# Beryl2000/SE-UNet-AirSeg

Hardware: AMD Instinct MI355X
Metric: voxels/sec SE-UNet fwd+bwd, 128^3 patch (higher is better)
Workload: dtype bf16

## Files before the change

include/seunet_hip.h:

```cpp
#ifndef SEUNET_HIP_H
#define SEUNET_HIP_H
#include <stddef.h>

#ifdef __cplusplus
extern "C" {
#endif

#ifndef SEUNET_F32
#define SEUNET_F32 0
#define SEUNET_BF16 1
#define SEUNET_F16 2
#endif
#define SEUNET_CONV_MFMA 0
#define SEUNET_CONV_NAIVE 1
#define SEUNET_CONV_MARCH 2
#define SEUNET_CONV_TILED 3

typedef void* seunet_stream_t;
typedef struct seunet_dims { int n, d, h, w; } seunet_dims;

int seunet_version(void);
const char* seunet_last_error(void);
int seunet_init(int device);

int seunet_pack_cl(int dtype, const float* in_ncdhw, int c, void* out_cl, int c_pad, seunet_dims dims, seunet_stream_t s);
int seunet_unpack_cl(int dtype, const void* in_cl, int c, float* out_ncdhw, seunet_dims dims, seunet_stream_t s);

size_t seunet_conv_wpack_bytes(int dtype, int taps, int cin, int cout);
int seunet_conv_pack_weights(int dtype, const float* w, int taps, int cin, int cout, int transpose_flip, void* wpack, seunet_stream_t s);
int seunet_conv_stats_slots(int impl, int taps, int dilation, seunet_dims dims);
int seunet_conv3d_fwd(int dtype, int impl, int taps, int dilation, int nsrc, const void* const* src, const int* src_c,
                      int cin, const void* weights, int transpose_flip, const float* bias, int ndst, void* const* dst,
                      const int* dst_c, const int* dst_accumulate, double* stats_partial, seunet_dims dims, seunet_stream_t s);
int seunet_conv3d_stream_supported(int dtype, int dilation, int src_c, int dst_c);
size_t seunet_conv3d_stream_wpack_bytes(int src_c);
int seunet_conv3d_stream_slots(int dilation, seunet_dims dims);
int seunet_conv3d_stream_pack(int dtype, const float* w, int cin_w, int cout_w, int transpose_flip, int src_c, int dst_c, void* wpack,
                              seunet_stream_t s);
int seunet_conv3d_stream(int dtype, int dilation, const void* src, int src_c, const void* wpack, const float* bias, void* dst, int dst_c,
                         int dst_accumulate, double* stats_partial, seunet_dims dims, seunet_stream_t s);
int seunet_conv3d_march_supported(int dtype, int dilation, int nsrc, const int* src_c, int ndst, const int* dst_c);
size_t seunet_conv3d_march_wpack_bytes(int cin, int cout);
int seunet_conv3d_march_slots(int dilation, int cin, int cout, seunet_dims dims);
int seunet_conv3d_march_pack(int dtype, const float* w, int cin_w, int cout_w, int transpose_flip, int cin, int cout, void* wpack,
                             seunet_stream_t s);
int seunet_conv3d_march(int dtype, int dilation, int nsrc, const void* const* src, const int* src_c, const void* wpack, const float* bias,
                        int ndst, void* const* dst, const int* dst_c, const int* dst_accumulate, double* stats_partial, seunet_dims dims,
                        seunet_stream_t s);
int seunet_conv3d_wgrad_stream_supported(int dtype, int dilation, int x_c, int dy_c);
size_t seunet_conv3d_wgrad_stream_workspace_bytes(int x_c, int dy_c, int dilation, seunet_dims dims);
int seunet_conv3d_wgrad_stream(int dtype, int dilation, const void* x, int x_c, int cin, const void* dy, int dy_c, int cout, float* dw,
                               void* workspace, size_t workspace_bytes, seunet_dims dims, seunet_stream_t s);
size_t seunet_conv3d_wgrad_workspace_bytes(int taps, int cin, int cout);
int seunet_conv3d_wgrad(int dtype, int impl, int taps, int dilation, int nsrc, const void* const* src, const int* src_c,
                        int cin, const void* dy, int cout, float* dw, void* workspace, size_t workspace_bytes,
                        seunet_dims dims, seunet_stream_t s);

int seunet_epilogue_slots(seunet_dims dims);
int seunet_channel_stats(int dtype, const void* t, int c, double* partial, seunet_dims dims, seunet_stream_t s);
int seunet_stats_finalize(const double* partial, int slots, int c, int n, long long count, float eps, int mode,
                          float* out_a, float* out_b, seunet_stream_t s);

int seunet_gate_epilogue_fwd(int dtype, const void* raw, const float* mean, const float* rstd, int c, const float* w_se,
                             const float* w_se2, const float* w_side, const float* b_side, float slope, void* e_out,
                             float* side_out, float* level_map, int level_accumulate, const float* head_w,
                             const float* drop, int drop_stride, seunet_dims dims, seunet_stream_t s);
int seunet_gate_epilogue_bwd(int dtype, const void* raw, const float* mean, const float* rstd, int c, const float* w_se,
                             const float* w_se2, const float* w_side, const float* b_side, float slope, const void* g_e,
                             const float* g_side, const float* g_level, const float* head_w, const float* drop,
                             int drop_stride, const float* m1, const float* m2, void* draw_out, double* stat_partial,
                             float* pgrad_partial, seunet_dims dims, seunet_stream_t s);
int seunet_pgrad_reduce(const float* pgrad_partial, int records, int c, float* dw_se, float* dw_se2, float* dw_side,
                        float* db_side, float* dhead_w, seunet_stream_t s);
int seunet_gate_bwd_finalize(const double* stat_partial, int slots, int c, int n, long long count, float* m1, float* m2,
                             const float* pgrad_partial, int records, float* dw_se, float* dw_se2, float* dw_side,
                             float* db_side, float* dhead_w, seunet_stream_t s);

int seunet_cat_epilogue_fwd(int dtype, const void* raw, const float* mean, const float* rstd, const void* raw2,
                            const float* mean2, const float* rstd2, int c, float slope, void* out, seunet_dims dims,
                            seunet_stream_t s);
int seunet_cat_epilogue_bwd(int dtype, const void* g_out, const void* raw, const float* mean, const float* rstd,
                            const void* raw2, const float* mean2, const float* rstd2, int c, float slope,
                            const float* m1, const float* m2, const float* m1b, const float* m2b, void* dx, void* dx2,
                            double* stat_partial, double* stat_partial2, seunet_dims dims, seunet_stream_t s);

int seunet_xbranch_moment_slots(seunet_dims dims);
int seunet_xbranch_moments(int dtype, const void* x_in, double* partial , seunet_dims dims, seunet_stream_t s);
int seunet_xbranch_stats(const double* partial, int slots, const float* w2, int c, int in_channel, int n, long long count,
                         float eps, float* mean2, float* rstd2, double* moments_out , seunet_stream_t s);
int seunet_cat_epilogue_fwd_x(int dtype, const void* raw, const float* mean, const float* rstd, const void* x_in,
                              const float* w2, int in_channel, const float* mean2, const float* rstd2, int c, float slope,
                              void* out, seunet_dims dims, seunet_stream_t s);
int seunet_cat_epilogue_bwd_x(int dtype, const void* g_out, const void* raw, const float* mean, const float* rstd,
                              const void* x_in, const float* w2, int in_channel, const float* mean2, const float* rstd2,
                              int c, float slope, const float* m1, const float* m2, const float* m1b, const float* m2b,
                              void* dx, double* stat_partial, double* stat_partial2, double* xw_partial, seunet_dims dims,
                              seunet_stream_t s);
int seunet_cat_epilogue_fwd_x_pool(int dtype, const void* raw, const float* mean, const float* rstd, const void* x_in,
                                   const float* w2, int in_channel, const float* mean2, const float* rstd2, int c, float slope,
                                   void* out, void* pooled, unsigned int* argmax, seunet_dims dims, seunet_stream_t s);
int seunet_cat_epilogue_bwd_x_pool(int dtype, const void* g_out, const void* raw, const float* mean, const float* rstd,
                                   const void* x_in, const float* w2, int in_channel, const float* mean2, const float* rstd2,
                                   int c, float slope, const float* m1, const float* m2, const float* m1b, const float* m2b,
                                   void* dx, double* stat_partial, double* stat_partial2, double* xw_partial,
                                   const unsigned int* pool_argmax, const void* pool_g, seunet_dims dims, seunet_stream_t s);
int seunet_cat_xgrad_finalize(const double* xw_partial, const double* stat_partial2, int slots, const double* moments,
                              const float* w2, int c, int in_channel, int n, float eps, float* dw, seunet_stream_t s);

int seunet_maxpool_fwd(int dtype, const void* in, int c, void* out, seunet_dims in_dims, seunet_stream_t s);
int seunet_maxpool_bwd(int dtype, const void* in, const void* g_out, int c, void* g_in, int accumulate,
                       seunet_dims in_dims, seunet_stream_t s);
int seunet_upsample2_fwd(int dtype, const void* in, int c, void* out, seunet_dims in_dims, seunet_stream_t s);
int seunet_upsample2_bwd(int dtype, const void* g_out, int c, void* g_in, int accumulate, seunet_dims in_dims,
                         seunet_stream_t s);
int seunet_side_upsample(const float* side, int c, int scale, float* out_ncdhw, int c_total, int c_off,
                         seunet_dims low_dims, seunet_stream_t s);

int seunet_head_fwd(const float* const* level_maps, int nlevels, const float* bias, float* pred, seunet_dims dims,
                    seunet_stream_t s);
size_t seunet_head_bwd_tmp_floats(seunet_dims dims);
int seunet_head_bwd(const float* g_pred, float* const* g_levels, int nlevels, float* tmp, float* g_bias,
                    seunet_dims dims, seunet_stream_t s);

#define SEUNET_LOSS_DICE 1
#define SEUNET_LOSS_GUL 2
#define SEUNET_LOSS_ATR 4
int seunet_loss_partial_floats(void);
int seunet_loss_sums(const float* pred, int apply_sigmoid, const float* target, const float* weight, const float* skel,
                     long long n, float* partial, double* sums, int terms, seunet_stream_t s);
int seunet_loss_value(const double* sums0, double c_dice0, double c_gul0, double c_atr0, const double* sums1, double c_dice1,
                      double c_gul1, double c_atr1, float* value, seunet_stream_t s);
int seunet_loss_grad(const float* pred, int apply_sigmoid, const float* target, const float* weight, const float* skel,
                     long long n, const double* sums, float c_dice, float c_gul, float c_atr, float g_scale,
                     const float* g_scale_dev, float* g_pred, seunet_stream_t s);

int seunet_loss_sample_partial_floats(int batch);
int seunet_loss_sums_per_sample(const float* pred, int apply_sigmoid, const float* target, const float* weight, const float* skel,
                                int batch, long long n_per_sample, float* partial, double* sums, int terms, seunet_stream_t s);
int seunet_loss_sample_values(const double* sums, int batch, double c_dice, double c_gul, double c_atr, float* values,
                              seunet_stream_t s);

size_t seunet_cldice_workspace_bytes(long long volumes, int n0, int n1, int n2, int iters, int save);
int seunet_cldice_partial_doubles(void);
int seunet_soft_skeleton(const float* x, long long volumes, int n0, int n1, int n2, int iters, float* out, int save, void* workspace,
                         size_t workspace_bytes, seunet_stream_t s);
int seunet_cldice_sums(const float* skel_pred, const float* target, const float* skel_target, const float* pred, long long n,
                       double* partial, double* sums, seunet_stream_t s);
int seunet_cldice_value(const double* sums, double smooth, float* value, double* scalars, seunet_stream_t s);
int seunet_cldice_backward(const float* target, const float* skel_target, const double* sums, double smooth, const float* g_dev,
                           long long volumes, int n0, int n1, int n2, int iters, float* grad, void* workspace, size_t workspace_bytes,
                           seunet_stream_t s);
int seunet_cldice_counts(const unsigned char* skel_pred, const unsigned char* label, const unsigned char* skel_label,
                         const unsigned char* pred, long long n, unsigned long long* counts, seunet_stream_t s);

int seunet_pool_select(const float* new_keys, int batch, float* keys, long long* seq, long long* state, int capacity, int* slots_out,
                       seunet_stream_t s);
int seunet_pool_scatter(const int* slots_dev, int batch, int capacity, long long voxels, const float* data, const float* label,
                        const float* weight, const float* skel, float* pool_data, unsigned char* pool_label, float* pool_weight,
                        unsigned char* pool_skel, seunet_stream_t s);
int seunet_pool_gather(const int* slots_host, int n, int capacity, long long voxels, const float* pool_data,
                       const unsigned char* pool_label, const float* pool_weight, const unsigned char* pool_skel, float* data_out,
                       float* label_out, float* weight_out, float* skel_out, seunet_stream_t s);

int seunet_adamw_step(float* const* params, const float* const* grads, float* const* exp_avg, float* const* exp_avg_sq,
                      const long long* counts, int n_tensors, double lr, double beta1, double beta2, double eps,
                      double weight_decay, int step, int maximize, seunet_stream_t s);
int seunet_adamw_step_gated(float* const* params, const float* const* grads, float* const* exp_avg, float* const* exp_avg_sq,
                            const long long* counts, const int* steps, float* const* skipped, int n_tensors, double lr,
                            double beta1, double beta2, double eps, double weight_decay, int maximize, const int* skip_flag,
                            float* table, seunet_stream_t s);

#define SEUNET_IMG_I16 0
#define SEUNET_IMG_F32 1
#define SEUNET_W_F16 0
#define SEUNET_W_F32 1
#define SEUNET_W_F64 2
int seunet_crop_batch(const void* img, int img_dtype, const unsigned char* label, const void* weight, int weight_dtype,
                      const unsigned char* skeleton, int d, int h, int w, int cube, int ncrop, const int* starts, const int* aug,
                      double weight_exponent, int f64_math, float* data_out, float* label_out, float* weight_out, float* skel_out,
                      seunet_stream_t s);
int seunet_hu_two_channel(const void* img, int img_dtype, long long nvox, int f64_math, float* out, seunet_stream_t s);

int seunet_window_gather(const float* volume, int c, int x, int y, int z, int cube, int nwin, const int* starts, float* out,
                         seunet_stream_t s);
int seunet_window_accumulate(const float* logits, int apply_sigmoid, int nwin, const int* starts, int cube, double* acc, int x, int y,
                             int z, seunet_stream_t s);
int seunet_window_finalize(const double* acc, int x, int y, int z, int cube, int nx, const int* xs, int ny, const int* ys, int nz,
                           const int* zs, int dup0, double* out, seunet_stream_t s);

#define SEUNET_DTI_F64 0
// ... 176 lines not shown
```

se-unet-airseg_amd/_lib.py:

```python
from __future__ import annotations

import ctypes as C
import os
from typing import Optional, Sequence

_HERE = os.path.dirname(os.path.abspath(__file__))
LIB_PATH = os.environ.get("SEUNET_LIB") or os.path.join(_HERE, "libseunet_hip.so")

F32, BF16, F16 = 0, 1, 2
CONV_MFMA, CONV_NAIVE, CONV_MARCH, CONV_TILED = 0, 1, 2, 3
LOSS_NSUMS = 7
DTI_F64, DTI_F32 = 0, 1
CC_EVALUATION, CC_MAXIMUM_3D, CC_LARGEST_FILLED = 0, 1, 2
MORPH_DILATE, MORPH_ERODE_BORDER0, MORPH_ERODE_BORDER1, MORPH_CLOSE = 0, 1, 2, 3


class Dims(C.Structure):
    _fields_ = [("n", C.c_int), ("d", C.c_int), ("h", C.c_int), ("w", C.c_int)]


class NetDesc(C.Structure):
    _fields_ = [("batch", C.c_int), ("in_channel", C.c_int), ("n_classes", C.c_int),
                ("d", C.c_int), ("h", C.c_int), ("w", C.c_int), ("width_mult", C.c_int),
                ("dtype", C.c_int), ("conv_impl", C.c_int),
# ... 1 lines not shown


KERNEL_NAIVE, KERNEL_TILED, KERNEL_STREAM, KERNEL_MARCH, KERNEL_WGRAD1X1 = range(5)
KERNEL_NAMES = ("Naive", "Tiled", "Stream", "March", "Wgrad1x1")


class ConvInfo(C.Structure):
    _fields_ = [("name", C.c_char * 16), ("taps", C.c_int), ("dilation", C.c_int), ("level", C.c_int), ("dims", Dims),
                ("nsrc", C.c_int), ("src_c", C.c_int * 3), ("src_is_input", C.c_int * 3), ("cin", C.c_int), ("cout", C.c_int),
                ("need_dgrad", C.c_int), ("fwd", C.c_int), ("dgrad", C.c_int), ("wgrad", C.c_int),
                ("x_name", C.c_char * 16), ("x_materialised", C.c_int), ("x_fwd", C.c_int), ("x_wgrad", C.c_int),
                ("src_dist", C.c_longlong)]


_vp, _i, _f, _ll, _sz, _d =C.c_void_p, C.c_int, C.c_float, C.c_longlong, C.c_size_t, C.c_double
_pp = C.POINTER(C.c_void_p)
_ip = C.POINTER(C.c_int)

PROTOTYPES = {
    "seunet_version": (_i, []),
    "seunet_last_error": (C.c_char_p, []),
    "seunet_pack_cl": (_i, [_i, _vp, _i, _vp, _i, Dims, _vp]),
    "seunet_unpack_cl": (_i, [_i, _vp, _i, _vp, Dims, _vp]),
    "seunet_conv_wpack_bytes": (_sz, [_i, _i, _i, _i]),
    "seunet_conv_pack_weights": (_i, [_i, _vp, _i, _i, _i, _i, _vp, _vp]),
    "seunet_conv_stats_slots": (_i, [_i, _i, _i, Dims]),
    "seunet_conv3d_fwd": (_i, [_i, _i, _i, _i, _i, _pp, _ip, _i, _vp, _i, _vp, _i, _pp, _ip, _ip, _vp, Dims, _vp]),
    "seunet_conv3d_stream_supported": (_i, [_i, _i, _i, _i]),
    "seunet_conv3d_stream_wpack_bytes": (_sz, [_i]),
    "seunet_conv3d_stream_slots": (_i, [_i, Dims]),
    "seunet_conv3d_stream_pack": (_i, [_i, _vp, _i, _i, _i, _i, _i, _vp, _vp]),
    "seunet_conv3d_stream": (_i, [_i, _i, _vp, _i, _vp, _vp, _vp, _i, _i, _vp, Dims, _vp]),
    "seunet_conv3d_march_supported": (_i, [_i, _i, _i, _ip, _i, _ip]),
    "seunet_conv3d_march_wpack_bytes": (_sz, [_i, _i]),
    "seunet_conv3d_march_slots": (_i, [_i, _i, _i, Dims]),
    "seunet_conv3d_march_pack": (_i, [_i, _vp, _i, _i, _i, _i, _i, _vp, _vp]),
    "seunet_conv3d_march": (_i, [_i, _i, _i, _pp, _ip, _vp, _vp, _i, _pp, _ip, _ip, _vp, Dims, _vp]),
    "seunet_conv3d_wgrad_stream_supported": (_i, [_i, _i, _i, _i]),
    "seunet_conv3d_wgrad_stream_workspace_bytes": (_sz, [_i, _i, _i, Dims]),
    "seunet_conv3d_wgrad_stream": (_i, [_i, _i, _vp, _i, _i, _vp, _i, _i, _vp, _vp, _sz, Dims, _vp]),
    "seunet_conv3d_wgrad_workspace_bytes": (_sz, [_i, _i, _i]),
    "seunet_conv3d_wgrad": (_i, [_i, _i, _i, _i, _i, _pp, _ip, _i, _vp, _i, _vp, _vp, _sz, Dims, _vp]),
    "seunet_epilogue_slots": (_i, [Dims]),
    "seunet_channel_stats": (_i, [_i, _vp, _i, _vp, Dims, _vp]),
    "seunet_stats_finalize": (_i, [_vp, _i, _i, _i, _ll, _f, _i, _vp, _vp, _vp]),
    "seunet_gate_epilogue_fwd": (_i, [_i, _vp, _vp, _vp, _i, _vp, _vp, _vp, _vp, _f, _vp, _vp, _vp, _i, _vp, _vp, _i, Dims, _vp]),
    "seunet_gate_epilogue_bwd": (_i, [_i, _vp, _vp, _vp, _i, _vp, _vp, _vp, _vp, _f, _vp, _vp, _vp, _vp, _vp, _i, _vp, _vp, _vp, _vp, _vp, Dims, _vp]),
    "seunet_pgrad_reduce": (_i, [_vp, _i, _i, _vp, _vp, _vp, _vp, _vp, _vp]),
    "seunet_gate_bwd_finalize": (_i, [_vp, _i, _i, _i, _ll, _vp, _vp, _vp, _i, _vp, _vp, _vp, _vp, _vp, _vp]),
    "seunet_cat_epilogue_fwd": (_i, [_i, _vp, _vp, _vp, _vp, _vp, _vp, _i, _f, _vp, Dims, _vp]),
    "seunet_cat_epilogue_bwd": (_i, [_i, _vp, _vp, _vp, _vp, _vp, _vp, _vp, _i, _f, _vp, _vp, _vp, _vp, _vp, _vp, _vp, _vp, Dims, _vp]),
    "seunet_maxpool_fwd": (_i, [_i, _vp, _i, _vp, Dims, _vp]),
    "seunet_maxpool_bwd": (_i, [_i, _vp, _vp, _i, _vp, _i, Dims, _vp]),
    "seunet_upsample2_fwd": (_i, [_i, _vp, _i, _vp, Dims, _vp]),
    "seunet_upsample2_bwd": (_i, [_i, _vp, _i, _vp, _i, Dims, _vp]),
    "seunet_side_upsample": (_i, [_vp, _i, _i, _vp, _i, _i, Dims, _vp]),
    "seunet_head_fwd": (_i, [_pp, _i, _vp, _vp, Dims, _vp]),
    "seunet_head_bwd_tmp_floats": (_sz, [Dims]),
    "seunet_head_bwd": (_i, [_vp, _pp, _i, _vp, _vp, Dims, _vp]),
    "seunet_loss_partial_floats": (_i, []),
    "seunet_loss_sums": (_i, [_vp, _i, _vp, _vp, _vp, _ll, _vp, _vp, _i, _vp]),
    "seunet_loss_value": (_i, [_vp, _d, _d, _d, _vp, _d, _d, _d, _vp, _vp]),
    "seunet_loss_grad": (_i, [_vp, _i, _vp, _vp, _vp, _ll, _vp, _f, _f, _f, _f, _vp, _vp, _vp]),
    "seunet_loss_sample_partial_floats": (_i, [_i]),
    "seunet_loss_sums_per_sample": (_i, [_vp, _i, _vp, _vp, _vp, _i, _ll, _vp, _vp, _i, _vp]),
    "seunet_loss_sample_values": (_i, [_vp, _i, _d, _d, _d, _vp, _vp]),
    "seunet_cldice_workspace_bytes": (_sz, [_ll, _i, _i, _i, _i, _i]),
    "seunet_cldice_partial_doubles": (_i, []),
    "seunet_soft_skeleton": (_i, [_vp, _ll, _i, _i, _i, _i, _vp, _i, _vp, _sz, _vp]),
    "seunet_cldice_sums": (_i, [_vp, _vp, _vp, _vp, _ll, _vp, _vp, _vp]),
    "seunet_cldice_value": (_i, [_vp, _d, _vp, _vp, _vp]),
    "seunet_cldice_backward": (_i, [_vp, _vp, _vp, _d, _vp, _ll, _i, _i, _i, _i, _vp, _vp, _sz, _vp]),
    "seunet_cldice_counts": (_i, [_vp, _vp, _vp, _vp, _ll, _vp, _vp]),
    "seunet_pool_select":(_i, [_vp, _i, _vp, _vp, _vp, _i, _vp, _vp]),
    "seunet_pool_scatter": (_i, [_vp, _i, _i, _ll, _vp, _vp, _vp, _vp, _vp, _vp, _vp, _vp, _vp]),
    "seunet_pool_gather": (_i, [_ip, _i, _i, _ll, _vp, _vp, _vp, _vp, _vp, _vp, _vp, _vp, _vp]),
    "seunet_xbranch_moment_slots": (_i, [Dims]),
    "seunet_xbranch_moments": (_i, [_i, _vp, _vp, Dims, _vp]),
    "seunet_xbranch_stats": (_i, [_vp, _i, _vp, _i, _i, _i, _ll, _f, _vp, _vp, _vp, _vp]),
    "seunet_cat_epilogue_fwd_x": (_i, [_i, _vp, _vp, _vp, _vp, _vp, _i, _vp, _vp, _i, _f, _vp, Dims, _vp]),
    "seunet_cat_epilogue_bwd_x": (_i, [_i, _vp, _vp, _vp, _vp, _vp, _vp, _i, _vp, _vp, _i, _f, _vp, _vp, _vp, _vp, _vp, _vp, _vp, _vp, Dims, _vp]),
    "seunet_cat_epilogue_fwd_x_pool": (_i, [_i, _vp, _vp, _vp, _vp, _vp, _i, _vp, _vp, _i, _f, _vp, _vp, _vp, Dims, _vp]),
    "seunet_cat_epilogue_bwd_x_pool": (_i, [_i, _vp, _vp, _vp, _vp, _vp, _vp, _i, _vp, _vp, _i, _f, _vp, _vp, _vp, _vp, _vp, _vp, _vp, _vp, _vp, _vp, Dims, _vp]),
    "seunet_cat_xgrad_finalize": (_i, [_vp, _vp, _i, _vp, _vp, _i, _i, _i, _f, _vp, _vp]),
    "seunet_cc_workspace_bytes": (_sz, [_i, _i, _i]),
    "seunet_largest_component": (_i, [_vp, _i, _i, _i, _i, _vp, _vp, _vp, _sz, _vp]),
    "seunet_metric_out_bytes": (_sz, [_i]),
    "seunet_metric_sums": (_i, [_vp, _vp, _vp, _vp, _ll, _i, _vp, _sz, _vp]),
    "seunet_value_counts": (_i, [_vp, _ll, _i, _vp, _vp]),
    "seunet_shift_clamp": (_i, [_vp, _ll, _i, _i, _i, _i, _vp, _vp]),
    "seunet_get_l_workspace_bytes": (_sz, [_i, _i, _i]),
    "seunet_get_l": (_i, [_vp, _i, _i, _i, _d, _i, _vp, _vp, _sz, _vp]),
    "seunet_mask_combine": (_i, [_vp, _vp, _ll, _i, _vp, _vp]),
    "seunet_mask_box": (_i, [_vp, _i, _i, _i, _vp, _vp]),
    "seunet_crop3d": (_i, [_vp, _i, _i, _i, _i, _ip, _vp, _vp]),
    "seunet_crop_batch": (_i, [_vp, _i, _vp, _vp, _i, _vp, _i, _i, _i, _i, _i, _ip, _ip, C.c_double, _i, _vp, _vp, _vp, _vp, _vp]),
    "seunet_hu_two_channel": (_i, [_vp, _i, _ll, _i, _vp, _vp]),
    "seunet_window_gather": (_i, [_vp, _i, _i, _i, _i, _i, _i, _ip, _vp, _vp]),
    "seunet_window_accumulate": (_i, [_vp, _i, _i, _ip, _i, _vp, _i, _i, _i, _vp]),
    "seunet_window_finalize": (_i, [_vp, _i, _i, _i, _i, _i, _ip, _i, _ip, _i, _ip, _i, _vp, _vp]),
    "seunet_dti_workspace_bytes": (_sz, [_i, _i, _i]),
    "seunet_dti": (_i, [_vp, _i, _i, _i, C.c_double, C.c_double, _i, _vp, _vp, _sz, _vp]),
    "seunet_edt_workspace_bytes": (_sz, [_i, _i, _i]),
    "seunet_edt": (_i, [_vp, _i, _i, _i, _vp, _vp, _vp, _vp, _vp, _sz, _vp]),
    "seunet_edt_sampling_workspace_bytes": (_sz, [_i, _i, _i]),
    "seunet_edt_sampling": (_i, [_vp, _i, _i, _i, _d, _d, _d, _vp, _vp, _vp, _vp, _vp, _sz, _vp]),
    "seunet_mask_bits": (_i, [_vp, _ll, _vp, _vp]),
    "seunet_hard_mining_masks": (_i, [_vp, _vp, _vp, _i, _i, _i, _vp, _vp, _vp]),
    "seunet_lib_weight_workspace_bytes": (_sz, [_i, _i, _i]),
    "seunet_lib_weight": (_i, [_vp, _i, _i, _i, _vp, _vp, _vp, _sz, _vp]),
    "seunet_break_weight_workspace_bytes": (_sz, [_i, _i, _i]),
    "seunet_break_weight": (_i, [_vp, _vp, _vp, _i, _i, _i, _vp, _vp, _vp, _vp, _sz, _vp]),
    "seunet_skeleton_workspace_bytes": (_sz, [_i, _i, _i]),
    "seunet_skeletonize": (_i, [_vp, _i, _i, _i, _vp, _vp, _vp, _sz, _vp]),
    "seunet_skeleton_branches_workspace_bytes": (_sz, [_i, _i, _i]),
    "seunet_skeleton_branches": (_i, [_vp, _i, _i, _i, _i, _vp, _vp, _vp, _vp, _sz, _vp]),
    "seunet_parse_assign_workspace_bytes": (_sz, [_i, _i, _i]),
    "seunet_parse_assign": (_i, [_vp, _vp, _vp, _i, _i, _i, _vp, _vp, _vp, _sz, _vp]),
    "seunet_label_stats_max_num": (_i, []),
    "seunet_label_stats": (_i, [_vp, _i, _i, _i, _i, _vp, _vp, _vp, _vp]),
    "seunet_relabel": (_i, [_vp, _ll, _vp, _i, _vp, _vp]),
    "seunet_binary_morph_workspace_bytes": (_sz, [_i, _i, _i]),
    "seunet_binary_morph": (_i, [_vp, _i, _i, _i, _i, _vp, _vp, _sz, _vp]),
    "seunet_fill_holes": (_i, [_vp, _i, _i, _i, _vp, _vp, _sz, _vp]),
    "seunet_slice_moments": (_i, [_vp, _i, _i, _i, _i, _vp, _vp]),
    "seunet_scatter_labels": (_i, [_vp, _vp, _ll, _ll, _vp, _vp, _vp, _vp]),
    "seunet_mesh_workspace_bytes": (_sz, [_i, _i, _i]),
    "seunet_mesh_count": (_i, [_vp, _i, _i, _i, C.POINTER(_ll), C.POINTER(_ll), _vp, _sz, _vp]),
    "seunet_mesh_emit": (_i, [_i, _i, _i, _d, _ll, _ll, _vp, _vp, _vp, _sz, _vp]),
    "seunet_mesh_label_workspace_bytes": (_sz, [_i, _i, _i]),
    "seunet_mesh_label_sort_bytes": (_sz, [_ll, _ll]),
    "seunet_mesh_label_count": (_i, [_vp, _i, _i, _i, _i, C.POINTER(_ll), C.POINTER(_ll), _ip, _ip, _vp, _vp, _i, _vp, _sz, _vp]),
    "seunet_mesh_label_emit": (_i, [_vp, _i, _i, _i, _i, _d, _ll, _ll, _vp, _vp, _vp, _sz, _vp, _sz, _vp]),
    "seunet_branch_stats": (_i, [_vp, _vp, _vp, _i, _i, _i, _i] + [_vp] * 11 + [_vp]),
    "seunet_branch_wall_stats": (_i, [_vp, _vp, _vp, _i, _i, _i, _i, _d, _d, _d, _vp, _vp, _vp, _vp, _vp, _vp]),
    "seunet_surface_workspace_bytes": (_sz, [_i, _i, _i]),
    "seunet_surface_count": (_i, [_vp, _vp, _i, _i, _i, C.POINTER(_ll), C.POINTER(_ll), _ip, _vp, _sz, _vp]),
    "seunet_surface_emit_workspace_bytes": (_sz, [_i, _i, _i]),
    "seunet_surface_emit": (_i, [_i, _i, _i, _ip, _d, _d, _d, _ll, _ll, _vp, _vp, _vp, _sz, _vp, _sz, _vp]),
    "seunet_surface_summary_bytes": (_sz, [_i]),
    "seunet_surface_summary": (_i, [_vp, _ll, _ll, C.POINTER(_d), _i, _vp, _vp]),
    "seunet_select_ranks_workspace_bytes": (_sz, [_i]),
    "seunet_select_ranks": (_i, [_vp, _ll, C.POINTER(_ll), C.POINTER(_ll), C.POINTER(_ll), _i, _vp, _vp, _sz, _vp]),
    "seunet_mesh_coord_sums": (_i, [_vp, _i, _i, _i, _vp, _vp]),
    "seunet_mesh_adjacency_workspace_bytes": (_sz, [_ll, _ll]),
    "seunet_mesh_adjacency": (_i, [_vp, _ll, _ll, _vp, _vp, _ll, _vp, _vp, _vp, _sz, _vp]),
    "seunet_mesh_smooth": (_i, [_vp, _ll, _vp, _vp, _vp, _i, _f, _vp, _vp, _vp]),
    "seunet_mesh_affine": (_i, [_vp, _ll, C.POINTER(_f), C.POINTER(_f), _vp, _vp]),
    "seunet_mesh_stl_records": (_i, [_vp, _ll, _vp, _ll, C.POINTER(_f), C.POINTER(_f), _vp, _vp, _vp]),
    "seunet_adamw_step": (_i, [_vp, _vp, _vp, _vp, _vp, _i, C.c_double, C.c_double, C.c_double, C.c_double, C.c_double, _i, _i, _vp]),
    "seunet_adamw_step_gated": (_i, [_vp, _vp, _vp, _vp, _vp, _vp, _vp, _i, C.c_double, C.c_double, C.c_double, C.c_double, C.c_double,
                                     _i, _vp, _vp, _vp]),
    "seunet_net_param_count": (_i, [C.POINTER(NetDesc)]),
    "seunet_net_param_info": (_i, [C.POINTER(NetDesc), _i, C.c_char_p, _i, _ip, _ip]),
    "seunet_net_workspace_bytes": (_sz, [C.POINTER(NetDesc)]),
    "seunet_net_forward": (_i, [C.POINTER(NetDesc), _pp, _vp, _vp, _vp, _vp, _vp, _vp, _sz, _vp]),
    "seunet_prof_enable": (_i, [_i]),
    "seunet_prof_enable_filtered": (_i, [C.c_char_p]),
    "seunet_prof_report": (_i, [C.c_char_p, _sz]),
    "seunet_init": (_i, [_i]),
    "seunet_net_forward_capture": (_i, [C.POINTER(NetDesc), _pp, _vp, _vp, _vp, _vp, _vp, _vp, _sz, _vp, C.POINTER(C.c_void_p)]),
    "seunet_graph_launch": (_i, [_vp, _vp]),
    "seunet_graph_destroy": (_i, [_vp]),
    "seunet_net_read_tensor": (_i, [C.POINTER(NetDesc), _pp, _vp, _sz, C.c_char_p, _i, _vp, _ip, _vp]),
    "seunet_net_conv_info": (_i, [C.POINTER(NetDesc), _i, C.POINTER(ConvInfo)]),
    "seunet_net_backward": (_i, [C.POINTER(NetDesc), _pp, _vp, _vp, _vp, _vp, _pp, _vp, _sz, _vp]),
# ... 63 lines not shown
```

se-unet-airseg_amd/csrc/abi.cpp:

```cpp
#include "seunet_common.h"
#include "epilogue.h"
#include "volume.h"
#include "wgrad.h"
#include "../../include/seunet_hip.h"

using namespace seunet;

static inline Dims D(seunet_dims d) { return Dims{d.n, d.d, d.h, d.w}; }
static inline hipStream_t S(seunet_stream_t s) { return reinterpret_cast<hipStream_t>(s); }

static int make_src(int nsrc, const void* const* src, const int* src_c, SrcList& l) {
  SEUNET_CHECK(nsrc >= 1 && nsrc <= 3 && src && src_c, "bad source list");
  l = SrcList{};
  l.n = nsrc;
  for (int i = 0; i < nsrc; ++i) { l.ptr[i] = src[i]; l.C[i] = src_c[i]; }
  return 0;
}

namespace seunet { extern unsigned long long* g_conv_debug; }

extern "C" {

int seunet_debug_set_buffer(void* p) { seunet::g_conv_debug = reinterpret_cast<unsigned long long*>(p); return 0; }
int seunet_debug_upsample2_form(int dtype, int c, seunet_dims dims, int backward) { return upsample2_form(dtype, c, D(dims), backward != 0); }
// ... 135 lines not shown
                        seunet_stream_t s) {
  SrcList sl;
  if (int e = make_src(nsrc, src, src_c, sl)) return e;
  SEUNET_CHECK(dy && dw, "conv3d_wgrad: null tensor");
  if (impl == SEUNET_CONV_NAIVE) return launch_wgrad_naive(dtype, taps, dilation, sl, cin, dy, cout, dw, D(dims), S(s));
  SEUNET_CHECK(workspace, "conv3d_wgrad: null workspace");
  const ConvKernel k = impl == SEUNET_CONV_MARCH ? (taps == 1 ? ConvKernel::Wgrad1x1 : ConvKernel::March)
                       : impl == SEUNET_CONV_TILED ? ConvKernel::Tiled
                                                   : wgrad_kernel(dtype, taps, dilation, sl, cin, cout, D(dims), sl.gap());
  return run_wgrad(k, dtype, taps, dilation, sl, cin, dy, cout, dw, workspace, workspace_bytes, D(dims), S(s));
}

int seunet_epilogue_slots(seunet_dims dims) { return epi_partials(D(dims)); }
int seunet_channel_stats(int dtype, const void* t, int c, double* partial, seunet_dims dims, seunet_stream_t s) {
  SEUNET_CHECK(t && partial, "channel_stats: null tensor");
  return launch_channel_stats(dtype, t, c, partial, D(dims), S(s));
}
int seunet_stats_finalize(const double* partial, int slots, int c, int n, long long count, float eps, int mode, float* out_a,
                          float* out_b, seunet_stream_t s) {
  SEUNET_CHECK(partial && out_a && out_b && slots >= 1 && count >= 1, "stats_finalize: bad argument");
  return launch_stats_finalize(partial, slots, c, n, count, eps, mode, out_a, out_b, S(s));
}

int seunet_gate_epilogue_fwd(int dtype, const void* raw, const float* mean, const float* rstd, int c, const float* w_se,
                             const float* w_se2, const float* w_side, const float* b_side, float slope, void* e_out,
                             float* side_out, float* level_map, int level_accumulate, const float* head_w, const float* drop,
                             int drop_stride, seunet_dims dims, seunet_stream_t s) {
  SEUNET_CHECK(raw && mean && rstd && w_se && w_side && b_side && e_out, "gate_epilogue_fwd: null tensor");
  SEUNET_CHECK(!level_map || head_w, "gate_epilogue_fwd: level_map needs head_w");
  const GateBlock b{{raw, mean, rstd}, c, {w_se, w_se2, w_side, b_side, slope}};
  SseHead h{side_out, level_map, level_accumulate, head_w, drop, drop_stride};
  return launch_sse_fwd(dtype, b, e_out, h, D(dims), S(s));
}
int seunet_gate_epilogue_bwd(int dtype, const void* raw, const float* mean, const float* rstd, int c, const float* w_se,
                             const float* w_se2, const float* w_side, const float* b_side, float slope, const void* g_e,
                             const float* g_side, const float* g_level, const float* head_w, const float* drop, int drop_stride,
                             const float* m1, const float* m2, void* draw_out, double* stat_partial, float* pgrad_partial,
                             seunet_dims dims, seunet_stream_t s) {
  SEUNET_CHECK(raw && mean && rstd && w_se && w_side && b_side, "gate_epilogue_bwd: null tensor");
  SEUNET_CHECK(!g_level || head_w, "gate_epilogue_bwd: g_level needs head_w");
  const GateBlock b{{raw, mean, rstd}, c, {w_se, w_se2, w_side, b_side, slope}};
  SseBwdIn g{g_e, g_side, g_level};
  SseHead h{nullptr, nullptr, 0, head_w, drop, drop_stride};
  if (m1 == nullptr) return launch_sse_bwd_sums(dtype, b, g, h, {stat_partial, pgrad_partial}, D(dims), S(s));
  return launch_sse_bwd_apply(dtype, b, g, h, {m1, m2, draw_out}, D(dims), S(s));
}
int seunet_pgrad_reduce(const float* pgrad_partial, int records, int c, float* dw_se, float* dw_se2, float* dw_side,
                        float* db_side, float* dhead_w, seunet_stream_t s) {
  SEUNET_CHECK(pgrad_partial && records >= 1, "pgrad_reduce: bad argument");
  return launch_pgrad_reduce(pgrad_partial, records, c, dw_se, dw_se2, dw_side, db_side, dhead_w, S(s));
}
int seunet_gate_bwd_finalize(const double* stat_partial, int slots, int c, int n, long long count, float* m1, float* m2,
                             const float* pgrad_partial, int records, float* dw_se, float* dw_se2, float* dw_side,
                             float* db_side, float* dhead_w, seunet_stream_t s) {
  SEUNET_CHECK(stat_partial && m1 && m2 && pgrad_partial && slots >= 1 && n >= 1 && count >= 1, "gate_bwd_finalize: bad argument");
  SEUNET_CHECK(c % 8 == 0 && c >= 8 && c <= 128 && (c & (c - 1)) == 0, "channel count %d must be a power of two in [8,128]", c);
  SEUNET_CHECK(records == n * slots, "gate_bwd_finalize: records=%d, pass A wrote n * slots = %d", records, n * slots);
  return launch_gate_bwd_finalize(stat_partial, slots, c, n, count, m1, m2, pgrad_partial, records, dw_se, dw_se2, dw_side,
                                  db_side, dhead_w, S(s));
}
static int cat_epilogue_bwd(int dtype, const CatBlock& b, const void* g_out, const PoolGrad& pool, const float* m1, const float* m2,
                            const float* m1b, const float* m2b, void* dx, void* dx2, double* stat_partial, double* stat_partial2,
                            double* xw_partial, seunet_dims dims, seunet_stream_t s) {
  if (m1 == nullptr) return launch_cat_bwd_sums(dtype, b, g_out, pool, {stat_partial, stat_partial2, xw_partial}, D(dims), S(s));
  return launch_cat_bwd_apply(dtype, b, g_out, pool, {m1, m2, m1b, m2b, dx, dx2, nullptr, 0}, D(dims), S(s));
}
int seunet_cat_epilogue_fwd(int dtype, const void* raw, const float* mean, const float* rstd, const void* raw2,
                            const float* mean2, const float* rstd2, int c, float slope, void* out, seunet_dims dims,
                            seunet_stream_t s) {
  SEUNET_CHECK(raw && mean && rstd && out && (!raw2 || (mean2 && rstd2)), "cat_epilogue_fwd: null tensor");
  const CatBlock b{{raw, mean, rstd}, {raw2 ? Branch2::Stored : Branch2::None, raw2, mean2, rstd2, nullptr, 0}, c, slope};
  return launch_cat_fwd(dtype, b, out, PoolOut{}, D(dims), S(s));
}
int seunet_cat_epilogue_bwd(int dtype, const void* g_out, const void* raw, const float* mean, const float* rstd,
                            const void* raw2, const float* mean2, const float* rstd2, int c, float slope, const float* m1,
                            const float* m2, const float* m1b, const float* m2b, void* dx, void* dx2, double* stat_partial,
                            double* stat_partial2, seunet_dims dims, seunet_stream_t s) {
  SEUNET_CHECK(g_out && raw && mean && rstd, "cat_epilogue_bwd: null tensor");
  SEUNET_CHECK(!raw2 || (mean2 && rstd2), "cat_epilogue_bwd: second branch incomplete");
  const CatBlock b{{raw, mean, rstd}, {raw2 ? Branch2::Stored : Branch2::None, raw2, mean2, rstd2, nullptr, 0}, c, slope};
  return cat_epilogue_bwd(dtype, b, g_out, PoolGrad{}, m1, m2, m1b, m2b, dx, dx2, stat_partial, stat_partial2, nullptr, dims, s);
}

int seunet_maxpool_fwd(int dtype, const void* in, int c, void* out, seunet_dims d, seunet_stream_t s) {
  SEUNET_CHECK(in && out, "maxpool_fwd: null tensor");
  return launch_maxpool_fwd(dtype, in, c, out, D(d), S(s));
}
int seunet_maxpool_bwd(int dtype, const void* in, const void* g_out, int c, void* g_in, int accumulate, seunet_dims d,
                       seunet_stream_t s) {
  SEUNET_CHECK(in && g_out && g_in, "maxpool_bwd: null tensor");
  return launch_maxpool_bwd(dtype, in, g_out, c, g_in, accumulate, D(d), S(s));
}
int seunet_upsample2_fwd(int dtype, const void* in, int c, void* out, seunet_dims d, seunet_stream_t s) {
  SEUNET_CHECK(in && out, "upsample2_fwd: null tensor");
  return launch_upsample2_fwd(dtype, in, c, out, D(d), S(s));
}
int seunet_upsample2_bwd(int dtype, const void* g_out, int c, void* g_in, int accumulate, seunet_dims d, seunet_stream_t s) {
  SEUNET_CHECK(g_out && g_in, "upsample2_bwd: null tensor");
  return launch_upsample2_bwd(dtype, g_out, c, g_in, accumulate, D(d), S(s));
}
int seunet_side_upsample(const float* side, int c, int scale, float* out, int c_total, int c_off, seunet_dims low,
                         seunet_stream_t s) {
  SEUNET_CHECK(side && out && scale >= 1, "side_upsample: bad argument");
  return launch_side_upsample(side, c, scale, out, c_total, c_off, D(low), S(s));
}

int seunet_head_fwd(const float* const* level_maps, int nlevels, const float* bias, float* pred, seunet_dims d, seunet_stream_t s) {
  SEUNET_CHECK(level_maps && bias && pred, "head_fwd: null tensor");
  return launch_head_fwd(level_maps, nlevels, bias, pred, D(d), S(s));
}
size_t seunet_head_bwd_tmp_floats(seunet_dims d) { return head_bwd_tmp_floats(D(d)); }
int seunet_head_bwd(const float* g_pred, float* const* g_levels, int nlevels, float* tmp, float* g_bias, seunet_dims d,
                    seunet_stream_t s) {
  SEUNET_CHECK(g_pred && g_levels && tmp, "head_bwd: null tensor");
  return launch_head_bwd(g_pred, g_levels, nlevels, tmp, g_bias, D(d), S(s));
}

int seunet_loss_partial_floats(void) { return loss_partials() * SEUNET_LOSS_NSUMS; }
int seunet_loss_sums(const float* pred, int apply_sigmoid, const float* target, const float* weight, const float* skel,
                     long long n, float* partial, double* sums, int terms, seunet_stream_t s) {
  SEUNET_CHECK(pred && target && partial && sums && n >= 1, "loss_sums: bad argument");
  SEUNET_CHECK(terms >= 0 && terms <= 7, "loss_sums: terms=%d is not a mask of SEUNET_LOSS_DICE | _GUL | _ATR", terms);
  return launch_loss_sums(pred, apply_sigmoid, target, weight, skel, n, partial, sums, S(s), terms);
}
int seunet_loss_value(const double* sums0, double c_dice0, double c_gul0, double c_atr0, const double* sums1, double c_dice1,
                      double c_gul1, double c_atr1, float* value, seunet_stream_t s) {
  SEUNET_CHECK(sums0 && value, "loss_value: null argument");
  return launch_loss_value(sums0, c_dice0, c_gul0, c_atr0, sums1, c_dice1, c_gul1, c_atr1, value, S(s));
}
int seunet_loss_grad(const float* pred, int apply_sigmoid, const float* target, const float* weight, const float* skel,
                     long long n, const double* sums, float c_dice, float c_gul, float c_atr, float g_scale,
                     const float* g_scale_dev, float* g_pred, seunet_stream_t s) {
  SEUNET_CHECK(pred && target && sums && g_pred && n >= 1, "loss_grad: bad argument");
  return launch_loss_grad(pred, apply_sigmoid, target, weight, skel, n, sums, c_dice, c_gul, c_atr, g_scale, g_scale_dev, g_pred, S(s));
}

int seunet_loss_sample_partial_floats(int batch) {
  if (batch < 1 || batch > 65535) { fail("loss_sample_partial_floats: batch %d (1..65535)", batch); return 0; }
  return loss_sample_partials(batch) * SEUNET_LOSS_NSUMS;
}
int seunet_loss_sums_per_sample(const float* pred, int apply_sigmoid, const float* target, const float* weight, const float* skel,
                                int batch, long long n_per_sample, float* partial, double* sums, int terms, seunet_stream_t s) {
  SEUNET_CHECK(pred && target && partial && sums && n_per_sample >= 1, "loss_sums_per_sample: bad argument");
  SEUNET_CHECK(batch >= 1 && batch <= 65535, "loss_sums_per_sample: batch %d (1..65535)", batch);
  SEUNET_CHECK(terms >= 0 && terms <= 7, "loss_sums_per_sample: terms=%d is not a mask of SEUNET_LOSS_DICE | _GUL | _ATR", terms);
  return launch_loss_sums_per_sample(pred, apply_sigmoid, target, weight, skel, batch, n_per_sample, partial, sums, terms, S(s));
}
int seunet_loss_sample_values(const double* sums, int batch, double c_dice, double c_gul, double c_atr, float* values, seunet_stream_t s) {
  SEUNET_CHECK(sums && values && batch >= 1, "loss_sample_values: bad argument");
  return launch_loss_sample_values(sums, batch, c_dice, c_gul, c_atr, values, S(s));
}

size_t seunet_cldice_workspace_bytes(long long volumes, int n0, int n1, int n2, int iters, int save) {
  if (volumes < 1 || n0 < 1 || n1 < 1 || n2 < 1) { fail("cldice_workspace_bytes: empty shape (%lld volumes of (%d, %d, %d))", volumes, n0, n1, n2); return 0; }
  if (iters < 0 || iters > kCldiceMaxIters) { fail("cldice_workspace_bytes: iters=%d (0..%d)", iters, kCldiceMaxIters); return 0; }
  if ((long long)n0 * n1 * n2 >= (1ll << 31) / volumes) { fail("cldice_workspace_bytes: fewer than 2^31 voxels in all supported"); return 0; }
  return cldice_workspace_bytes(volumes, n0, n1, n2, iters, save != 0);
}
int seunet_cldice_partial_doubles(void) { return cldice_partial_doubles(); }
int seunet_soft_skeleton(const float* x, long long volumes, int n0, int n1, int n2, int iters, float* out, int save, void* workspace,
                         size_t workspace_bytes, seunet_stream_t s) {
  return launch_soft_skeleton(x, volumes, n0, n1, n2, iters, out, save != 0, workspace, workspace_bytes, S(s));
}
int seunet_cldice_sums(const float* skel_pred, const float* target, const float* skel_target, const float* pred, long long n,
                       double* partial, double* sums, seunet_stream_t s) {
  return launch_cldice_sums(skel_pred, target, skel_target, pred, n, partial, sums, S(s));
// ... 378 lines not shown
```

se-unet-airseg_amd/csrc/cat.hip:

```cpp
#include "epilogue.h"
#include "wgrad.h"
#include <type_traits>

namespace seunet {

template <bool XR>
__device__ __forceinline__ void second_branch(const float (&in8)[8], const float (&wa)[8], const float (&wb)[8], float (&x2)[8]) {
#pragma unroll
  for (int j = 0; j < 8; ++j) x2[j] = XR ? wa[j] * in8[0] + wb[j] * in8[1] : in8[j];
}

template <typename T, int LPV, bool TWO, bool XR>
__global__ void __launch_bounds__(EPI_THREADS)
cat_fwd_kernel(const T* __restrict__ raw, const float* __restrict__ mean, const float* __restrict__ rstd,
               const T* __restrict__ raw2, const float* __restrict__ mean2, const float* __restrict__ rstd2, int C, float slope,
               T* __restrict__ out, long long V, const float* __restrict__ w2x, int xic) {
  SEUNET_EPI_THREAD(LPV);
  float mu[8], rs[8], mu2[8], rs2[8], wa[8], wb[8];
#pragma unroll
  for (int j = 0; j < 8; ++j) {
    mu[j] = mean[n * C + c0 + j]; rs[j] = rstd[n * C + c0 + j];
    mu2[j] = TWO ? mean2[n * C + c0 + j] : 0.f;
    rs2[j] = TWO ? rstd2[n * C + c0 + j] : 0.f;
    wa[j] = XR ? w2x[(c0 + j) * xic] : 0.f;
// ... 4 lines not shown
  Pack8<T> nx, nx2;
  zero8p(nx); zero8p(nx2);
  if (v < V) {
    const long long o = ((long long)n * V + v) * C + c0;
    load8p(raw + o, nx);
    if (TWO) load8p(XR ? raw2 + ((long long)n * V + v) * 8 : raw2 + o, nx2);
  }
  for (; v < V; v += stride) {
    const long long o = ((long long)n * V + v) * C + c0;
    float x[8], in2[8], x2[8], y[8];
    unpack8(nx, x);
    if (TWO) { unpack8(nx2, in2); second_branch<XR>(in2, wa, wb, x2); }
    if (v + stride < V) {
      load8p(raw + o + stride * C, nx);
      if (TWO) load8p(XR ? raw2 + ((long long)n * V + v + stride) * 8 : raw2 + o + stride * C, nx2);
    }
#pragma unroll
    for (int j = 0; j < 8; ++j) y[j] = norm_lrelu(x[j], mu[j], rs[j], slope);
    if (TWO) {
#pragma unroll
      for (int j = 0; j < 8; ++j) y[j] += norm_lrelu(x2[j], mu2[j], rs2[j], slope);
    }
    store8(out + o, y);
  }
}

template <typename T, int LPV>
__global__ void __launch_bounds__(EPI_THREADS)
cat_fwd_pool_kernel(const T* __restrict__ raw, const float* __restrict__ mean, const float* __restrict__ rstd,
                    const T* __restrict__ xin, const float* __restrict__ mean2, const float* __restrict__ rstd2, int C, float slope,
                    T* __restrict__ out, T* __restrict__ pooled, int D, int H, int W, const float* __restrict__ w2x, int xic,
                    unsigned* __restrict__ argmax) {
  SEUNET_EPI_THREAD(LPV);
  float mu[8], rs[8], mu2[8], rs2[8], wa[8], wb[8];
#pragma unroll
  for (int j = 0; j < 8; ++j) {
    mu[j] = mean[n * C + c0 + j]; rs[j] = rstd[n * C + c0 + j];
    mu2[j] = mean2[n * C + c0 + j]; rs2[j] = rstd2[n * C + c0 + j];
    wa[j] = w2x[(c0 + j) * xic];
    wb[j] = xic > 1 ? w2x[(c0 + j) * xic + 1] : 0.f;
  }
  const int Do = D / 2, Ho = H / 2, Wo = W / 2;
  const long long V = (long long)D * H * W, Vo = (long long)Do * Ho * Wo;
  const long long stride = (long long)P * VPB;
  for (long long cv = (long long)blockIdx.x * VPB + vb; cv < Vo; cv += stride) {
    const int xo = (int)(cv % Wo);
    const int yo = (int)((cv / Wo) % Ho);
    const int zo = (int)(cv / ((long long)Wo * Ho));
    const long long v0 = ((long long)(2 * zo) * H + 2 * yo) * W + 2 * xo;
    Pack8<T> px[8], pi[8];
#pragma unroll
    for (int k = 0; k < 8; ++k) {
      const long long v = v0 + ((long long)(k >> 2) * H + ((k >> 1) & 1)) * W + (k & 1);
      load8p(raw + ((long long)n * V + v) * C + c0, px[k]);
      load8p(xin + ((long long)n * V + v) * 8, pi[k]);
    }
    float m[8];
    unsigned am = 0;
#pragma unroll
    for (int j = 0; j < 8; ++j) m[j] = -INFINITY;
#pragma unroll
    for (int k = 0; k < 8; ++k) {
      const long long v = v0 + ((long long)(k >> 2) * H + ((k >> 1) & 1)) * W + (k & 1);
      float x[8], in2[8], x2[8], y[8];
      unpack8(px[k], x);
      unpack8(pi[k], in2);
      second_branch<true>(in2, wa, wb, x2);
#pragma unroll
      for (int j = 0; j < 8; ++j) y[j] = norm_lrelu(x[j], mu[j], rs[j], slope);
#pragma unroll
      for (int j = 0; j < 8; ++j) y[j] += norm_lrelu(x2[j], mu2[j], rs2[j], slope);
      store8(out + ((long long)n * V + v) * C + c0, y);
#pragma unroll
      for (int j = 0; j < 8; ++j) {
        const float yr = round_to<T>(y[j]);
        if (yr > m[j]) { m[j] = yr; am = (am & ~(7u << (3 * j))) | ((unsigned)k << (3 * j)); }
      }
    }
    store8(pooled + ((long long)n * Vo + cv) * C + c0, m);
    if (argmax != nullptr) argmax[((long long)n * Vo + cv) * (C / 8) + cg] = am;
  }
}

struct PoolRef {
  const unsigned* argmax;
  const void* g_pool;
  unsigned W, H, Wo, Ho;
  unsigned mW, mH;
  long long Vo;
};
__device__ __forceinline__ unsigned div_small(unsigned n, unsigned d, unsigned m, unsigned& rem) {
  unsigned q = __umulhi(n, m);
  unsigned r = n - q * d;
  if (r >= d) { ++q; r -= d; }
  rem = r;
  return q;
}
__device__ __forceinline__ void pool_locate(const PoolRef& pr, unsigned v, unsigned& kpos, unsigned& cv) {
  unsigned x, y;
  const unsigned t = div_small(v, pr.W, pr.mW, x);
  const unsigned z = div_small(t, pr.H, pr.mH, y);
  kpos = ((z & 1u) << 2) | ((y & 1u) << 1) | (x & 1u);
  cv = ((z >> 1) * pr.Ho + (y >> 1)) * pr.Wo + (x >> 1);
}

template <typename T, int LPV, bool TWO, bool APPLY, bool XW, bool XR, bool XG>
__global__ void __launch_bounds__(EPI_THREADS)
cat_bwd_kernel(const T* g_out, const T* __restrict__ raw, const float* __restrict__ mean, const float* __restrict__ rstd,
               const T* __restrict__ raw2, const float* __restrict__ mean2, const float* __restrict__ rstd2, int C, float slope,
               const float* __restrict__ m1p, const float* __restrict__ m2p, const float* __restrict__ m1bp,
               const float* __restrict__ m2bp, T* dxhat_out, T* dxhat2_out, double* __restrict__ stat_partial,
               double* __restrict__ stat_partial2, long long V, double* __restrict__ xw_partial, const float* __restrict__ w2x,
               int xic, PoolRef pool, float* __restrict__ gx_out, int gx_acc) {
  static_assert(!XG || (APPLY && XR), "XG: pass B of an XR block only");
  static_assert(!XW || XR, "XW: the weight-gradient sums are formed from the recomputed branch's own input voxel");
  SEUNET_EPI_THREAD(LPV);
  const bool pooled = pool.argmax != nullptr;
  const unsigned* pam = pool.argmax + (long long)n * pool.Vo * (C / 8) + cg;
  const T* pgp = reinterpret_cast<const T*>(pool.g_pool) + (long long)n * pool.Vo * C + c0;
  float mu[8], rs[8], mu2[8], rs2[8], a1[8], a2[8], b1[8], b2[8];
  typedef typename std::conditional<sizeof(T) == 2, float, double>::type SumT;
  SumT s[4][8];
  SumT xw[8][2];
  float wa[8], wb[8];
#pragma unroll
  for (int j = 0; j < 8; ++j) {
    xw[j][0] = xw[j][1] = 0.0;
    wa[j] = XR ? w2x[(c0 + j) * xic] : 0.f;
    wb[j] = (XR && xic > 1) ? w2x[(c0 + j) * xic + 1] : 0.f;
  }
#pragma unroll
  for (int j = 0; j < 8; ++j) {
    mu[j] = mean[n * C + c0 + j]; rs[j] = rstd[n * C + c0 + j];
    mu2[j] = TWO ? mean2[n * C + c0 + j] : 0.f;
    rs2[j] = TWO ? rstd2[n * C + c0 + j] : 0.f;
    a1[j] = APPLY ? m1p[n * C + c0 + j] : 0.f;
    a2[j] = APPLY ? m2p[n * C + c0 + j] : 0.f;
    b1[j] = (APPLY && TWO) ? m1bp[n * C + c0 + j] : 0.f;
    b2[j] = (APPLY && TWO) ? m2bp[n * C + c0 + j] : 0.f;
    s[0][j] = s[1][j] = s[2][j] = s[3][j] = 0.0;
  }
  const long long stride = (long long)P * VPB;
  long long v = (long long)blockIdx.x * VPB + vb;
  Pack8<T> ng, nx, nx2, npg;
  unsigned nam = 0, nkpos = 0;
  zero8p(ng); zero8p(nx); zero8p(nx2); zero8p(npg);
  auto fetch_pool = [&](long long vv) __attribute__((always_inline)) {
    unsigned cv;
    pool_locate(pool, (unsigned)vv, nkpos, cv);
    nam = pam[(long long)cv * (C / 8)];
    load8p(pgp + (long long)cv * C, npg);
  };
  if (v < V) {
    const long long o = ((long long)n * V + v) * C + c0;
    load8p(g_out + o, ng);
    load8p(raw + o, nx);
    if (TWO) load8p(XR ? raw2 + ((long long)n * V + v) * 8 : raw2 + o, nx2);
    if (pooled) fetch_pool(v);
  }
  for (; v < V; v += stride) {
    const long long o = ((long long)n * V + v) * C + c0;
    float gy[8], x[8], in2[8], x2[8], d[8];
    unpack8(ng, gy);
    unpack8(nx, x);
    if (TWO) { unpack8(nx2, in2); second_branch<XR>(in2, wa, wb, x2); }
    if (pooled) {
      float gp[8];
      unpack8(npg, gp);
#pragma unroll
      for (int j = 0; j < 8; ++j) gy[j] += ((nam >> (3 * j)) & 7u) == nkpos ? gp[j] : 0.f;
    }
    if (v + stride < V) {
      load8p(g_out + o + stride * C, ng);
      load8p(raw + o + stride * C, nx);
      if (TWO) load8p(XR ? raw2 + ((long long)n * V + v + stride) * 8 : raw2 + o + stride * C, nx2);
      if (pooled) fetch_pool(v + stride);
    }
#pragma unroll
    for (int j = 0; j < 8; ++j) {
      const float xh = (x[j] - mu[j]) * rs[j];
      d[j] = gy[j] * lrelu_slope(xh, slope);
      if (APPLY) d[j] = rs[j] * (d[j] - a1[j] - xh * a2[j]);
      else { s[0][j] += (SumT)d[j]; s[1][j] += (SumT)d[j] * (SumT)xh; }
    }
    if (TWO) {
      float d2[8];
#pragma unroll
// ... 135 lines not shown
      const double rs2 = 1.0 / (var + eps), rs = sqrt(rs2);
      const double proj = wa * A0 + wb * A1;
      g0 += rs * (A0 - rs2 * proj * (wa * c00 + wb * c01));
      g1 += rs * (A1 - rs2 * proj * (wa * c01 + wb * c11));
    }
    __syncthreads();
  }
  if (threadIdx.x == 0) {
    dw[c * ic] = (float)g0;
    if (ic > 1) dw[c * ic + 1] = (float)g1;
  }
}
__global__ void __launch_bounds__(256)
xw_finalize_kernel(const double* __restrict__ xw_partial, const double* __restrict__ stat_partial2, int slots, int C, int N,
                   const double* __restrict__ moments, const float* __restrict__ w2, int ic, double eps, float* __restrict__ dw) {
  xw_finalize_body(blockIdx.x, xw_partial, stat_partial2, slots, C, N, moments, w2, ic, eps, dw);
}
__global__ void __launch_bounds__(256)
cat_bwd_finalize_kernel(const double* __restrict__ partial, const double* __restrict__ partial2, int slots, int C, int N,
                        double inv_count, float* __restrict__ m1, float* __restrict__ m2, float* __restrict__ m1b,
                        float* __restrict__ m2b, int nb2, int nxw, const double* __restrict__ xw_partial,
                        const double* __restrict__ moments, const float* __restrict__ w2, int ic, double eps, float* __restrict__ dw,
                        WgReduceJob rider) {
  const int b = blockIdx.x, nb = N * C;
  if (b < nb) stats_finalize_body(b, partial, slots, C, inv_count, 0.f, 1, m1, m2);
  else if (b < nb + nb2) stats_finalize_body(b - nb, partial2, slots, C, inv_count, 0.f, 1, m1b, m2b);
  else if (b < nb + nb2 + nxw) xw_finalize_body(b - nb - nb2, xw_partial, partial2, slots, C, N, moments, w2, ic, eps, dw);
  else wgrad_reduce_body(rider, b - nb - nb2 - nxw);
}

template <typename T>
__global__ void __launch_bounds__(256)
xbranch_values_kernel(const T* __restrict__ x_in, const float* __restrict__ w2x, int C, int xic, float* __restrict__ out, long long V,
                      long long total) {
  for (long long i = blockIdx.x * (long long)blockDim.x + threadIdx.x; i < total; i += (long long)gridDim.x * blockDim.x) {
    const int cg = (int)(i % (C / 8));
    const long long nv = i / (C / 8);
    const long long n = nv / V, v = nv % V;
    float wa[8], wb[8], in2[8], x2[8];
#pragma unroll
    for (int j = 0; j < 8; ++j) {
      wa[j] = w2x[(cg * 8 + j) * xic];
      wb[j] = xic > 1 ? w2x[(cg * 8 + j) * xic + 1] : 0.f;
    }
    Pack8<T> px;
    load8p(x_in + nv * 8, px);
    unpack8(px, in2);
    second_branch<true>(in2, wa, wb, x2);
#pragma unroll
    for (int j = 0; j < 8; ++j) out[(n * C + cg * 8 + j) * V + v] = x2[j];
  }
}

static int cat_branch(const char* who, const CatBlock& b, Branch2& x, bool& two, bool& xr) {
  if (int e = check_c(b.C)) return e;
  x = b.b.kind == Branch2::None ? Branch2{} : b.b;
  two = x.kind != Branch2::None;
  xr = x.kind == Branch2::Recomputed;
  SEUNET_CHECK(!xr || (x.in_channel >= 1 && x.in_channel <= 2), "%s: in_channel %d (1 or 2)", who, x.in_channel);
  return 0;
}

int launch_cat_fwd(int dtype, const CatBlock& b, void* out, const PoolOut& pool, Dims d, hipStream_t s) {
  Branch2 x;
  bool two, xr;
  if (int e = cat_branch("cat_epilogue_fwd", b, x, two, xr)) return e;
  SEUNET_CHECK(!pool.pooled || (xr && d.D % 2 == 0 && d.H % 2 == 0 && d.W % 2 == 0),
               "cat_epilogue_fwd: the fused max-pool needs a recomputed second branch and even extents");
  dim3 grid(epi_partials(d) * 4, d.N);
#define SEUNET_CAT_FWD(...) <<<grid, EPI_THREADS, 0, s>>>((const T*)b.a.raw, b.a.mean, b.a.rstd, (const T*)x.src, x.mean2, x.rstd2, b.C, b.slope, (T*)out, __VA_ARGS__)
  SEUNET_LPV_SWITCH(b.C / 8, {
    SEUNET_DTYPE_SWITCH(dtype, {
      if (pool.pooled) cat_fwd_pool_kernel<T, LPV> SEUNET_CAT_FWD((T*)pool.pooled, d.D, d.H, d.W, x.w2, x.in_channel, pool.argmax);
      else if (xr) cat_fwd_kernel<T, LPV, true, true> SEUNET_CAT_FWD(d.vox(), x.w2, x.in_channel);
      else if (two) cat_fwd_kernel<T, LPV, true, false> SEUNET_CAT_FWD(d.vox(), nullptr, 0);
      else cat_fwd_kernel<T, LPV, false, false> SEUNET_CAT_FWD(d.vox(), nullptr, 0);
    });
  });
#undef SEUNET_CAT_FWD
  SEUNET_LAUNCH_CHECK();
  return 0;
}

static int cat_bwd_pool(const char* who, bool xr, const PoolGrad& pool, Dims d, PoolRef& pr) {
  pr = PoolRef{};
  if (pool.argmax == nullptr) return 0;
  SEUNET_CHECK(xr && pool.g_pool != nullptr && d.D % 2 == 0 && d.H % 2 == 0 && d.W % 2 == 0 && d.vox() < (1ll << 31),
               "%s: pooled gradient needs a recomputed second branch and even extents below 2^31 voxels", who);
  pr.argmax = pool.argmax; pr.g_pool = pool.g_pool;
  pr.W = (unsigned)d.W; pr.H = (unsigned)d.H; pr.Wo = (unsigned)d.W / 2; pr.Ho = (unsigned)d.H / 2;
  pr.mW = (unsigned)((1ull << 32) / (unsigned)d.W); pr.mH = (unsigned)((1ull << 32) / (unsigned)d.H);
  pr.Vo = d.vox() / 8;
  return 0;
}

#define SEUNET_CAT_BWD(TWO, APPLY, XW, XR, XG)                                                                                   \
  cat_bwd_kernel<T, LPV, TWO, APPLY, XW, XR, XG><<<grid, EPI_THREADS, 0, s>>>(                                                    \
      (const T*)g_out, (const T*)b.a.raw, b.a.mean, b.a.rstd, (const T*)x.src, x.mean2, x.rstd2, b.C, b.slope, a.m1, a.m2, a.m1b, \
      a.m2b, (T*)a.dx, (T*)a.dx2, o.stat_partial, o.stat_partial2, d.vox(), o.xw_partial, x.w2, x.in_channel, pr, a.gx_out,     \
      a.gx_acc)

int launch_cat_bwd_sums(int dtype, const CatBlock& b, const void* g_out, const PoolGrad& pool, const CatSums& out, Dims d,
                        hipStream_t s) {
  Branch2 x;
  bool two, xr;
  PoolRef pr;
  if (int e = cat_branch("cat_epilogue_bwd_sums", b, x, two, xr)) return e;
  if (int e = cat_bwd_pool("cat_epilogue_bwd_sums", xr, pool, d, pr)) return e;
  SEUNET_CHECK(out.stat_partial && (!two || out.stat_partial2), "cat_epilogue_bwd_sums needs the partial buffers");
  SEUNET_CHECK(!out.xw_partial || xr, "cat_epilogue_bwd_sums: the weight-gradient sums belong to a recomputed second branch");
  const CatSums o{out.stat_partial, two ? out.stat_partial2 : nullptr, out.xw_partial};
  const CatApply a{};
  dim3 grid(epi_partials(d), d.N);
  SEUNET_LPV_SWITCH(b.C / 8, {
    SEUNET_DTYPE_SWITCH(dtype, {
      if (xr && o.xw_partial) SEUNET_CAT_BWD(true, false, true, true, false);
      else if (xr) SEUNET_CAT_BWD(true, false, false, true, false);
      else if (two) SEUNET_CAT_BWD(true, false, false, false, false);
      else SEUNET_CAT_BWD(false, false, false, false, false);
    });
  });
  SEUNET_LAUNCH_CHECK();
  return 0;
}

int launch_cat_bwd_apply(int dtype, const CatBlock& b, const void* g_out, const PoolGrad& pool, const CatApply& io, Dims d,
                         hipStream_t s) {
  Branch2 x;
  bool two, xr;
  PoolRef pr;
  if (int e = cat_branch("cat_epilogue_bwd_apply", b, x, two, xr)) return e;
  if (int e = cat_bwd_pool("cat_epilogue_bwd_apply", xr, pool, d, pr)) return e;
  SEUNET_CHECK(io.m1 && io.m2 && io.dx && (!two || (io.m1b && io.m2b)) && (!two || xr || io.dx2),
               "cat_epilogue_bwd_apply: missing argument");
  SEUNET_CHECK(!io.gx_out || xr, "cat_epilogue_bwd_apply: the input-gradient term belongs to a recomputed second branch");
  const CatApply a{io.m1, io.m2, two ? io.m1b : nullptr, two ? io.m2b : nullptr, io.dx, two && !xr ? io.dx2 : nullptr,
                   io.gx_out, io.gx_out ? io.gx_acc : 0};
  const CatSums o{};
  dim3 grid(epi_partials(d) * 4, d.N);
  SEUNET_LPV_SWITCH(b.C / 8, {
    SEUNET_DTYPE_SWITCH(dtype, {
      if (xr && a.gx_out) SEUNET_CAT_BWD(true, true, false, true, true);
      else if (xr) SEUNET_CAT_BWD(true, true, false, true, false);
      else if (two) SEUNET_CAT_BWD(true, true, false, false, false);
      else SEUNET_CAT_BWD(false, true, false, false, false);
    });
  });
  SEUNET_LAUNCH_CHECK();
  return 0;
}
#undef SEUNET_CAT_BWD

int xbranch_moment_slots(Dims d) { return epi_partials(d); }

int launch_xbranch_moments(int dtype, const void* x_in, double* partial, Dims d, hipStream_t s) {
  dim3 grid(xbranch_moment_slots(d), d.N);
  SEUNET_DTYPE_SWITCH(dtype, input_moments_kernel<T><<<grid, EPI_THREADS, 0, s>>>((const T*)x_in, partial, d.vox()));
  SEUNET_LAUNCH_CHECK();
  return 0;
}

int launch_xbranch_stats(const double* partial, int slots, const float* w2, int C, int in_channel, int N, long long count,
                         float eps, float* mean2, float* rstd2, double* moments_out, hipStream_t s) {
  SEUNET_CHECK(in_channel >= 1 && in_channel <= 2, "xbranch_stats: in_channel %d (1 or 2)", in_channel);
  xbranch_stats_kernel<<<N, 256, 0, s>>>(partial, slots, w2, C, in_channel, 1.0 / (double)count, eps, mean2, rstd2, moments_out);
  SEUNET_LAUNCH_CHECK();
  return 0;
// ... 36 lines not shown
```

se-unet-airseg_amd/csrc/epilogue.h:

```cpp
#pragma once
#include "seunet_common.h"

namespace seunet {

struct WgReduceJob;
int epi_partials(Dims d);
int launch_channel_stats(int dtype, const void* t, int C, double* partial, Dims d, hipStream_t s);
int launch_stats_finalize(const double* partial, int slots, int C, int N, long long count,
                          float eps, int mode, float* out_a, float* out_b, hipStream_t s);
struct NormIn { const void* raw; const float* mean; const float* rstd; };
struct SseParams {
  const float* w_se;
  const float* w_se2;
  const float* w_side;
  const float* b_side;
  float slope;
};
struct GateBlock { NormIn a; int C; SseParams p; };
struct SseHead {
  float* side_out;
  float* level_map;
  int level_accumulate;
  const float* head_w;
  const float* drop;
  int drop_stride;
};
struct SseBwdIn {
  const void* g_e;
  const float* g_side;
  const float* g_level;
};
struct SseSums { double* stat_partial; float* pgrad_partial; };
struct SseApply { const float* m1; const float* m2; void* draw_out; };
int launch_sse_fwd(int dtype, const GateBlock& b, void* e_out, const SseHead& head, Dims d, hipStream_t s);
int launch_sse_bwd_sums(int dtype, const GateBlock& b, const SseBwdIn& g, const SseHead& head, const SseSums& out, Dims d,
                        hipStream_t s);
int launch_sse_bwd_apply(int dtype, const GateBlock& b, const SseBwdIn& g, const SseHead& head, const SseApply& io, Dims d,
                         hipStream_t s);
int launch_gate_bwd_finalize(const double* stat_partial, int slots, int C, int N, long long count, float* m1, float* m2,
                             const float* pgrad_partial, int records, float* dw_se, float* dw_se2, float* dw_side,
                             float* db_side, float* dhead_w, hipStream_t s, const WgReduceJob* rider = nullptr);
int launch_pgrad_reduce(const float* pgrad_partial, int records, int C, float* dw_se,
                        float* dw_se2, float* dw_side, float* db_side, float* dhead_w,
                        hipStream_t s);
struct Branch2 {
  enum Kind { None, Stored, Recomputed } kind;
  const void* src;
  const float* mean2;
  const float* rstd2;
  const float* w2;
  int in_channel;
};
struct CatBlock { NormIn a; Branch2 b; int C; float slope; };
struct PoolOut { void* pooled; unsigned* argmax; };
struct PoolGrad { const unsigned* argmax; const void* g_pool; };
struct CatSums {
  double* stat_partial;
  double* stat_partial2;
  double* xw_partial;
};
struct CatApply {
  const float *m1, *m2, *m1b, *m2b;
  void* dx;
  void* dx2;
  float* gx_out;
  int gx_acc;
};
int launch_cat_fwd(int dtype, const CatBlock& b, void* out, const PoolOut& pool, Dims d, hipStream_t s);
int launch_cat_bwd_sums(int dtype, const CatBlock& b, const void* g_out, const PoolGrad& pool, const CatSums& out, Dims d,
                        hipStream_t s);
int launch_cat_bwd_apply(int dtype, const CatBlock& b, const void* g_out, const PoolGrad& pool, const CatApply& io, Dims d,
                         hipStream_t s);
int xbranch_moment_slots(Dims d);
int launch_xbranch_moments(int dtype, const void* x_in, double* partial, Dims d, hipStream_t s);
int launch_xbranch_stats(const double* partial, int slots, const float* w2, int C, int in_channel, int N, long long count,
                         float eps, float* mean2, float* rstd2, double* moments_out, hipStream_t s);
int launch_cat_xgrad_finalize(const double* xw_partial, const double* stat_partial2, int slots, const double* moments, const float* w2,
                              int C, int in_channel, int N, float eps, float* dw, hipStream_t s);
struct CatXwFinalize { const double* xw_partial; const double* moments; const float* w2; int in_channel; float eps; float* dw; };
int launch_cat_bwd_finalize(const double* stat_partial, const double* stat_partial2, int slots, int C, int N, long long count,
                            float* m1, float* m2, float* m1b, float* m2b, const CatXwFinalize& xw, hipStream_t s,
                            const WgReduceJob* rider = nullptr);
int launch_xbranch_values(int dtype, const void* x_in, const float* w2, int C, int in_channel, float* out_ncdhw, Dims d, hipStream_t s);

#ifdef __HIPCC__
static constexpr int EPI_THREADS = 256;

template <typename T> __device__ __forceinline__ float round_to(float v) {
  if constexpr (sizeof(T) == 4) return v;
  else return unpack_lo<T>(pack2<T>(v, 0.f));
}

template <typename T> __device__ __forceinline__ float gate_sigmoid(float z) {
  if constexpr (sizeof(T) == 4) return 1.f / (1.f + expf(-z));
  else return __builtin_amdgcn_rcpf(1.f + __builtin_amdgcn_exp2f(-1.44269504088896341f * z));
}

#define SEUNET_EPI_THREAD(LPV)                                \
  const int n = blockIdx.y, P = gridDim.x;                    \
  const int cg = threadIdx.x % LPV, vb = threadIdx.x / LPV;   \
  constexpr int VPB = EPI_THREADS / LPV;                      \
  const int c0 = cg * 8

__device__ __forceinline__ float lrelu(float xh, float slope) { return xh > 0.f ? xh : xh * slope; }
__device__ __forceinline__ float norm_lrelu(float x, float mu, float rs, float slope) { return lrelu((x - mu) * rs, slope); }
__device__ __forceinline__ float lrelu_slope(float xh, float slope) { return xh > 0.f ? 1.f : slope; }

template <typename E, int K> __device__ __forceinline__ E wave4_sum(const E (&red)[4][16][K], int g, int k) {
  return ((red[0][g][k] + red[1][g][k]) + red[2][g][k]) + red[3][g][k];
}
template <typename E, int K> __device__ __forceinline__ E wave4_sum(const E (&red)[4][K], int k) {
  return ((red[0][k] + red[1][k]) + red[2][k]) + red[3][k];
}
template <typename E> __device__ __forceinline__ E wave4_sum(const E (&w)[4]) { return ((w[0] + w[1]) + w[2]) + w[3]; }

template <int K> __device__ __forceinline__ void block_sum(const double (&s)[K], double (&red)[4][K]) {
  const int wave = threadIdx.x >> 6, lane = threadIdx.x & 63;
#pragma unroll
  for (int k = 0; k < K; ++k) {
    double r = s[k];
#pragma unroll
    for (int off = 32; off >= 1; off >>= 1) r += shfl_xor_settled(r, off);
    if (lane == 0) red[wave][k] = r;
  }
  __syncthreads();
}

__device__ __forceinline__ void stats_finalize_body(int idx, const double* __restrict__ partial, int slots, int C, double inv_count,
                                                    float eps, int mode, float* __restrict__ out_a, float* __restrict__ out_b) {
  const int n = idx / C, c = idx % C;
  double s1 = 0.0, s2 = 0.0;
  for (int p = threadIdx.x; p < slots; p += 256) {
    const double* q = partial + (((long long)n * slots + p) * C + c) * 2;
    s1 += q[0];
    s2 += q[1];
  }
#pragma unroll
  for (int off = 32; off >= 1; off >>= 1) {
    s1 += shfl_xor_settled(s1, off);
    s2 += shfl_xor_settled(s2, off);
  }
  __shared__ double w1[4], w2[4];
  if ((threadIdx.x & 63) == 0) { w1[threadIdx.x >> 6] = s1; w2[threadIdx.x >> 6] = s2; }
  __syncthreads();
  if (threadIdx.x == 0) {
    s1 = wave4_sum(w1);
    s2 = wave4_sum(w2);
    if (mode == 0) {
      const double mean = s1 * inv_count;
      double var = s2 * inv_count - mean * mean;
      if (var < 0.0) var = 0.0;
      out_a[idx] = (float)mean;
      out_b[idx] = (float)(1.0 / sqrt(var + (double)eps));
    } else {
      out_a[idx] = (float)(s1 * inv_count);
      out_b[idx] = (float)(s2 * inv_count);
    }
  }
}

#define SEUNET_LPV_SWITCH(LPVVAL, ...)                                                  \
  switch (LPVVAL) {                                                                       \
    case 1: { constexpr int LPV = 1; __VA_ARGS__; } break;                                       \
    case 2: { constexpr int LPV = 2; __VA_ARGS__; } break;                                       \
    case 4: { constexpr int LPV = 4; __VA_ARGS__; } break;                                       \
    case 8: { constexpr int LPV = 8; __VA_ARGS__; } break;                                       \
    case 16: { constexpr int LPV = 16; __VA_ARGS__; } break;                                     \
    default: return fail("unsupported channel count %d (need 8,16,32,64 or 128)", (LPVVAL)*8); \
  }

static int check_c(int C) {
  SEUNET_CHECK(C % 8 == 0 && C >= 8 && C <= 128 && (C & (C - 1)) == 0, "channel count %d must be a power of two in [8,128]", C);
  return 0;
}
#endif

}
```

se-unet-airseg_amd/csrc/net.cpp:

```cpp
#include "seunet_common.h"
#include "epilogue.h"
#include "wgrad.h"
#include "../../include/seunet_hip.h"

#include <algorithm>
#include <cstdio>
#include <cstring>
#include <string>
#include <vector>

namespace seunet {

ConvKernel wgrad_kernel(int dtype, int taps, int dil, const SrcList& x, int cin_logical, int cout, Dims d, long long src_dist) {
  if (taps == 1) {
    const int combos = cdiv(cin_logical, 32) * cdiv(cout, 32);
    const long long nv = (long long)d.N * d.vox();
    const bool pays = combos >= 16 || (combos >= 8 && nv >= 500000);
    return pays && wgrad_1x1_supported(dtype, x, cin_logical, cout) ? ConvKernel::Wgrad1x1 : ConvKernel::Tiled;
  }
  const bool fine = d.W >= 32 && (long long)d.D * d.H * d.W >= 48LL * 48 * 48;
  const bool pays = fine || dil == 2 || cin_logical >= 256;
  return pays && wgrad_march_supported(dtype, taps, dil, x, cin_logical, cout, d, src_dist) ? ConvKernel::March : ConvKernel::Tiled;
}

namespace {

bool g_wgrad_defer = true;

enum TId {
  T_NONE,
  T_X0, T_X1, T_X2,
  T_E0, T_E1A, T_E1_1, T_E1, T_E2IN, T_E2, T_E3A, T_E3_1, T_E3, T_E4IN, T_E4, T_E5A, T_E5_1, T_E5,
  T_E6IN, T_E6, T_E7A, T_E7_1, T_E7, T_E8, T_D0A, T_D0_1, T_D0, T_D1U, T_D1A, T_D1_1, T_D1, T_D2U, T_D2A, T_D2_1,
  T_COUNT
};
enum OpKind { OP_GATED, OP_CAT, OP_POOL, OP_UP };
struct OpDesc {
  OpKind kind; const char* name;
  int src[3]; int dst;
  int cout;
  int dil; int gates;
  const char* xname; int xsrc;
};
constexpr OpDesc kOps[] = {
    {.kind = OP_GATED, .name = "ec1", .src = {T_X0}, .dst = T_E0, .cout = 8, .dil = 1, .gates = 1},
    {.kind = OP_GATED, .name = "ec2", .src = {T_E0}, .dst = T_E1A, .cout = 16, .dil = 1, .gates = 1},
    {.kind = OP_GATED, .name = "ec3", .src = {T_E1A}, .dst = T_E1_1, .cout = 32, .dil = 2, .gates = 1},
    {.kind = OP_CAT, .name = "ec33", .src = {T_E1_1, T_E0, T_E1A}, .dst = T_E1, .cout = 32, .xname = "x33", .xsrc = T_X0},
    {.kind = OP_POOL, .name = "pool0", .src = {T_E1}, .dst = T_E2IN},
    {.kind = OP_POOL, .name = "pool0x", .src = {T_X0}, .dst = T_X1},
    {.kind = OP_GATED, .name = "ec4", .src = {T_E2IN}, .dst = T_E2, .cout = 32, .dil = 1, .gates = 2},
    {.kind = OP_GATED, .name = "ec5", .src = {T_E2}, .dst = T_E3A, .cout = 32, .dil = 2, .gates = 2},
    {.kind = OP_GATED, .name = "ec6", .src = {T_E3A}, .dst = T_E3_1, .cout = 64, .dil = 2, .gates = 2},
    {.kind = OP_CAT, .name = "ec63", .src = {T_E3_1, T_E2, T_E3A}, .dst = T_E3, .cout = 64, .xname = "x63", .xsrc = T_X1},
    {.kind = OP_POOL, .name = "pool1", .src = {T_E3}, .dst = T_E4IN},
    {.kind = OP_POOL, .name = "pool1x", .src = {T_X1}, .dst = T_X2},
    {.kind = OP_GATED, .name = "ec7", .src = {T_E4IN}, .dst = T_E4, .cout = 64, .dil = 1, .gates = 2},
    {.kind = OP_GATED, .name = "ec8", .src = {T_E4}, .dst = T_E5A, .cout = 64, .dil = 2, .gates = 2},
    {.kind = OP_GATED, .name = "ec9", .src = {T_E5A}, .dst = T_E5_1, .cout = 64, .dil = 2, .gates = 2},
    {.kind = OP_CAT, .name = "ec93", .src = {T_E5_1, T_E4, T_E5A}, .dst = T_E5, .cout = 64, .xname = "x93", .xsrc = T_X2},
    {.kind = OP_POOL, .name = "pool2", .src = {T_E5}, .dst = T_E6IN},
    {.kind = OP_GATED, .name = "ec10", .src = {T_E6IN}, .dst = T_E6, .cout = 64, .dil = 1, .gates = 2},
    {.kind = OP_GATED, .name = "ec11", .src = {T_E6}, .dst = T_E7A, .cout = 64, .dil = 1, .gates = 2},
    {.kind = OP_GATED, .name = "ec12", .src = {T_E7A}, .dst = T_E7_1, .cout = 64, .dil = 1, .gates = 2},
    {.kind = OP_CAT, .name = "ec123", .src = {T_E7_1, T_E6, T_E7A}, .dst = T_E7, .cout = 64},
    {.kind = OP_UP, .name = "up0", .src = {T_E7}, .dst = T_E8},
    {.kind = OP_GATED, .name = "dc1", .src = {T_E8, T_E5}, .dst = T_D0A, .cout = 64, .dil = 1, .gates = 2},
    {.kind = OP_GATED, .name = "dc2", .src = {T_D0A}, .dst = T_D0_1, .cout = 64, .dil = 1, .gates = 2},
    {.kind = OP_CAT, .name = "dc22", .src = {T_D0_1, T_D0A}, .dst = T_D0, .cout = 64},
    {.kind = OP_UP, .name = "up1", .src = {T_D0}, .dst = T_D1U},
    {.kind = OP_GATED, .name = "dc3", .src = {T_D1U, T_E3}, .dst = T_D1A, .cout = 64, .dil = 1, .gates = 2},
    {.kind = OP_GATED, .name = "dc4", .src = {T_D1A}, .dst = T_D1_1, .cout = 32, .dil = 1, .gates = 2},
    {.kind = OP_CAT, .name = "dc42", .src = {T_D1_1, T_D1A}, .dst = T_D1, .cout = 32},
    {.kind = OP_UP, .name = "up2", .src = {T_D1}, .dst = T_D2U},
    {.kind = OP_GATED, .name = "dc5", .src = {T_D2U, T_E1}, .dst = T_D2A, .cout = 32, .dil = 1, .gates = 1},
    {.kind = OP_GATED, .name = "dc6", .src = {T_D2A}, .dst = T_D2_1, .cout = 16, .dil = 1, .gates = 1},
};
constexpr int kNumOps = sizeof(kOps) / sizeof(kOps[0]);
constexpr bool is_conv(const OpDesc& o) { return o.kind == OP_GATED || o.kind == OP_CAT; }

enum PField { P_CONV1_W, P_CONV1_B, P_CONV2_W, P_CONV2_B, P_SE, P_SE2, P_HEAD_W, P_HEAD_B };
constexpr const char* kFieldName[] = {"conv1.weight", "conv1.bias", "conv2.weight", "conv2.bias", "conv_se.weight", "conv_se2.weight",
                                      "weight", "bias"};
struct BlockParams { int at[6] = {-1, -1, -1, -1, -1, -1}, xw = -1; };
struct ParamDesc { const char* block; PField f; int cin, cout, k; };
constexpr int kNumParams = 117;

struct Graph {
  int level[T_COUNT] = {}, cbase[T_COUNT] = {};
  const char* tname[T_COUNT] = {};
  int nsrc[kNumOps] = {}, cin[kNumOps] = {};
  int head[kNumOps] = {}, slot[kNumOps] = {};
  int sides[2] = {};
  int first_up = -1, nconv = 0;
  BlockParams prm[kNumOps] = {};
  ParamDesc param[kNumParams] = {};
  int nparams = 0, dead = -1, head_w[2] = {}, head_b[2] = {};

  constexpr int add(const char* block, PField f, int ci, int co, int k) { param[nparams] = {block, f, ci, co, k}; return nparams++; }
  constexpr BlockParams add_block(const char* name, int gates, int ci, int co) {
    BlockParams b;
    const int fields = gates ? 4 + gates : 1;
    for (int f = 0; f < fields; ++f) b.at[f] = add(name, (PField)f, ci, co, gates ? 3 : 1);
    return b;
  }
};
constexpr Graph derive() {
  Graph g;
  g.tname[T_X0] = "x";
  for (int i = 0; i < kNumOps; ++i) {
    const OpDesc& o = kOps[i];
    for (int k = 0; k < 3 && o.src[k] != T_NONE; ++k) { ++g.nsrc[i]; g.cin[i] += g.cbase[o.src[k]]; }
    g.level[o.dst] = g.level[o.src[0]] + (o.kind == OP_POOL) - (o.kind == OP_UP);
    g.cbase[o.dst] = is_conv(o) ? o.cout : g.cbase[o.src[0]];
    g.tname[o.dst] = o.name;
    if (o.kind == OP_UP && g.first_up < 0) g.first_up = i;
    if (o.kind == OP_GATED) { g.head[i] = g.first_up >= 0; g.slot[i] = g.sides[g.head[i]]++; }
    if (!is_conv(o)) continue;
    ++g.nconv;
    g.prm[i] = g.add_block(o.name, o.gates, g.cin[i], o.cout);
    if (o.xname) g.prm[i].xw = g.add_block(o.xname, 0, 0, o.cout).at[P_CONV1_W];
  }
  g.dead = g.add_block("dc62", 0, 48, 16).at[P_CONV1_W];
  for (int h = 0; h < 2; ++h) {
    g.head_w[h] = g.add(h ? "dc0_1" : "dc0_0", P_HEAD_W, 2 * g.sides[h], 0, 1);
    g.head_b[h] = g.add(h ? "dc0_1" : "dc0_0", P_HEAD_B, 0, 0, 0);
  }
  return g;
}
constexpr Graph kG = derive();
static_assert(2 * kG.sides[0] == 24 && 2 * kG.sides[1] == 12, "dc0_0 takes 24 side channels, dc0_1 12 (SE_UNet.py:150-151)");
static_assert(kG.nparams == kNumParams, "the reference's state_dict has 117 tensors");

constexpr bool is_input(int t) { return kG.cbase[t] == 0; }

inline bool march_level(const Dims& d, int dil) {
  return d.W >= 32 && (d.vox() >= 48LL * 48 * 48 || (dil == 2 && d.vox() >= 32LL * 32 * 32));
}

int conv_slots(ConvKernel k, const Dims& dm, int taps, int dil, int cin, int cout) {
  switch (k) {
    case ConvKernel::Stream: return conv_stream_slots(dm, dil);
    case ConvKernel::March: return conv_march_slots(dm, dil, cin, cout);
    case ConvKernel::Naive: return epi_partials(dm);
    default: return conv_stats_tiles(dm, taps, dil);
  }
}

struct OpRes {
  size_t raw = 0, raw2 = 0, mean = 0, rstd = 0, mean2 = 0, rstd2 = 0, xtot = 0, wp_f = 0, wp_d = 0, wp_x = 0;
  int cin = 0, cout = 0, taps = 0;
  bool need_dgrad = false;
  ConvKernel fwd = ConvKernel::Tiled, dgrad = ConvKernel::Tiled, wgrad = ConvKernel::Tiled;
  ConvKernel x_fwd = ConvKernel::Tiled, x_wgrad = ConvKernel::Tiled;
  int fused = -1;
  size_t pool_idx = 0;
  size_t side = 0;
};

struct Take { const char* what; const char* of; size_t off, bytes; };
constexpr const char* kDigit[] = {"0", "1", "2", "3"};

struct Plan {
  seunet_net_desc d;
  size_t esz;
  Dims dims[4];
  int C[T_COUNT];
  size_t feat[T_COUNT], grad[T_COUNT];
  OpRes op[kNumOps];
  size_t lvl[2][4], glvl[2][4];
  size_t stats, stats2, pgrad, m1, m2, m1b, m2b, wgrad_ws, head_tmp, gx, xwp = 0, xmom = 0;
  size_t gside = 0, cls_part = 0, cls_bias = 0;
  bool fuse_x = false;
  size_t wgrad_ws_bytes;
  size_t total;
  size_t ig_gx[3] = {0, 0, 0}, ig_total = 0;

  size_t cur = 0;
  std::vector<Take> log;
  size_t take(size_t bytes, const char* what, const char* of = "") {
    log.push_back({what, of, cur, bytes});
    cur = align_up(cur + bytes, 256);
    return log.back().off;
  }

  const Dims& dims_of(int t) const { return dims[kG.level[t]]; }
  long long src_dist(int i) const {
    return kG.nsrc[i] == 2 ? (long long)feat[kOps[i].src[1]] - (long long)feat[kOps[i].src[0]] : 0;
  }

  void route(int i) {
    const OpDesc& o = kOps[i];
    OpRes& r = op[i];
    if (d.conv_impl == SEUNET_CONV_NAIVE) { r.fwd = r.dgrad = r.wgrad = r.x_fwd = r.x_wgrad = ConvKernel::Naive; return; }
    const Dims& dm = dims_of(o.dst);
    SrcList x{}, gy{};
    DstList y{}, gx{};
    x.n = gx.n = kG.nsrc[i];
    for (int k = 0; k < x.n; ++k) x.C[k] = gx.C[k] = C[o.src[k]];
    y.n = gy.n = 1;
    y.C[0] = gy.C[0] = r.cout;
    const int c0 = C[o.src[0]];
    const bool stream_ok = o.kind == OP_GATED && x.n == 1 && (long long)dm.D * dm.H * dm.W * 32 * (long long)esz < 0xFFFFFFFFll;
    const bool stream_f = stream_ok && conv_stream_supported(d.dtype, 27, o.dil, c0, r.cout);
    const bool stream_d = stream_ok && conv_stream_supported(d.dtype, 27, o.dil, r.cout, c0);
    const bool march_ok = o.kind == OP_GATED && !stream_f && march_level(dm, o.dil);
    r.fwd = stream_f ? ConvKernel::Stream
          : march_ok && conv_march_supported(d.dtype, 27, o.dil, x, y) ? ConvKernel::March : ConvKernel::Tiled;
    r.dgrad = stream_d ? ConvKernel::Stream
            : march_ok && conv_march_supported(d.dtype, 27, o.dil, gy, gx) ? ConvKernel::March : ConvKernel::Tiled;
    r.wgrad = stream_ok && wgrad_stream_supported(d.dtype, 27, o.dil, c0, r.cout)
                  ? ConvKernel::Stream : wgrad_kernel(d.dtype, r.taps, o.dil, x, r.cin, r.cout, dm, src_dist(i));
    if (o.xname) {
      const SrcList xs{{}, {8}, 1};
      r.x_fwd = ConvKernel::Tiled;
      r.x_wgrad = wgrad_kernel(d.dtype, 1, 1, xs, d.in_channel, r.cout, dm, 0);
    }
  }
  size_t wpack_bytes(ConvKernel k, int taps, int src_c, int cin, int cout) const {
    switch (k) {
      case ConvKernel::Stream: return conv_stream_wpack_bytes(src_c);
      case ConvKernel::March: return conv_march_wpack_bytes(cin, cout);
      default: return conv_wpack_bytes(d.dtype, taps, cin, cout);
    }
  }

  int init(const seunet_net_desc& desc) {
    d = desc;
    SEUNET_CHECK(d.batch >= 1 && d.in_channel >= 1 && d.in_channel <= 8, "net: batch/in_channel out of range");
    SEUNET_CHECK(d.n_classes >= 1 && d.n_classes <= class_max(), "net: n_classes=%d out of range (1 .. %d)", d.n_classes, class_max());
    SEUNET_CHECK(d.d % 8 == 0 && d.h % 8 == 0 && d.w % 8 == 0 && d.d >= 8 && d.h >= 8 && d.w >= 8,
                 "net: spatial extents (%d,%d,%d) must be multiples of 8", d.d, d.h, d.w);
    SEUNET_CHECK(d.width_mult == 1 || d.width_mult == 2, "net: width_mult %d unsupported (1 or 2)", d.width_mult);
    SEUNET_CHECK(dtype_ok(d.dtype), "net: dtype %d unsupported (SEUNET_F32 | SEUNET_BF16 | SEUNET_F16)", d.dtype);
    esz = dtype_size(d.dtype);
    log.reserve(320);
    for (int l = 0; l < 4; ++l) dims[l] = Dims{d.batch, d.d >> l, d.h >> l, d.w >> l};
    for (int t = T_X0; t < T_COUNT; ++t) C[t] = is_input(t) ? 8 : kG.cbase[t] * d.width_mult;
    auto tensor_bytes = [&](int t) { return (size_t)d.batch * dims_of(t).vox() * C[t] * esz; };
    static_assert(T_E1 < T_D2U, "the mate is placed before the walk reaches it");
    for (int t = T_X0; t < T_COUNT; ++t) {
      if (t != T_D2U) feat[t] = take(tensor_bytes(t), "out", kG.tname[t]);
      if (t == T_E1) feat[T_D2U] = take(tensor_bytes(T_D2U), "out", kG.tname[T_D2U]);
      grad[t] = is_input(t) ? 0 : take(tensor_bytes(t), "grad", kG.tname[t]);
    }
    size_t gx_max = 0, wg_max = 0, xw_max = 0, xmom_max = 0;
    fuse_x = d.in_channel <= 2 && d.conv_impl != SEUNET_CONV_NAIVE;
    int slots_max = 1, cmax = 8;
    for (int i = 0; i < kNumOps; ++i) {
      const OpDesc& o = kOps[i];
      OpRes& r = op[i];
      for (int c = 0; c < i && o.kind == OP_POOL && fuse_x; ++c) {
        if (kOps[c].kind != OP_CAT || !kOps[c].xname || kOps[c].dst != o.src[0]) continue;
        r.pool_idx = take((size_t)d.batch * dims_of(o.dst).vox() * (C[o.src[0]] / 8) * 4, "argmax", o.name);
        r.fused = c;
        op[c].fused = i;
      }
      if (!is_conv(o)) continue;
      const Dims& dm = dims_of(o.dst);
      r.cout = C[o.dst];
      r.taps = o.kind == OP_GATED ? 27 : 1;
      r.cin = kG.cin[i] ? kG.cin[i] * d.width_mult : d.in_channel;
      r.need_dgrad = kG.cin[i] != 0;
      const size_t act = tensor_bytes(o.dst);
      r.raw = take(act, "raw", o.name);
      r.mean = take((size_t)d.batch * r.cout * 4, "mean", o.name);
      r.rstd = take((size_t)d.batch * r.cout * 4, "rstd", o.name);
      route(i);
      r.wp_f = take(wpack_bytes(r.fwd, r.taps, C[o.src[0]], r.cin, r.cout), "wp_f", o.name);
      if (r.need_dgrad) r.wp_d = take(wpack_bytes(r.dgrad, r.taps, r.cout, r.cout, r.cin), "wp_d", o.name);
      slots_max = std::max(slots_max, conv_slots(r.fwd, dm, r.taps, o.dil, r.cin, r.cout));
      if (r.wgrad == ConvKernel::Stream) wg_max = std::max(wg_max, wgrad_stream_workspace_bytes(C[o.src[0]], r.cout, o.dil, dm));
      wg_max = std::max(wg_max, wgrad_workspace_bytes(r.taps, r.cin, r.cout));
// ... 326 lines not shown
    }
    if (!r.need_dgrad) return 0;
    const SrcList gsrc{{at(p.grad[o.dst])}, {r.cout}, 1};
    DstList gd{};
    gd.n = x.n;
    for (int k = 0; k < x.n; ++k) {
      const int t = o.src[k];
      gd.C[k] = p.C[t];
      gd.ptr[k] = is_input(t) ? nullptr : at(p.grad[t]);
      gd.acc[k] = (!is_input(t) && written[t]) ? 1 : 0;
      if (!is_input(t)) written[t] = true;
    }
    mark("dgrad:", o.name);
    return run_conv(r.dgrad, r.taps, o.dil, gsrc, r.cout, par(c.i, P_CONV1_W), 1, at(r.wp_d), nullptr, gd, nullptr, c.dm);
  }

  int heads_backward() {
    const Dims d1{1, p.dims[0].D, p.dims[0].H, p.dims[0].W};
    mark("head_bwd");
    for (int h = 0; h < 2; ++h) {
      const int nl = 4 - h;
      float* gb = grads[kG.head_b[h]];
      if (p.d.n_classes > 1) {
        if (int e = per_sample_class(p.glvl[h], 1, nl, [&](float* const* gl, size_t nc) {
              return launch_head_bwd(g_pred[h] + nc * d1.vox(), gl, nl, fat(p.head_tmp), fat(p.cls_bias) + nc, d1, s);
            })) return e;
        if (gb)
          if (int e = launch_class_bias_grad(fat(p.cls_bias), p.d.batch, p.d.n_classes, gb, s)) return e;
      } else {
        float* gl[4] = {nullptr, fat(p.glvl[h][1]), fat(p.glvl[h][2]), nl == 4 ? fat(p.glvl[h][3]) : nullptr};
        if (int e = launch_head_bwd(g_pred[h], gl, nl, fat(p.head_tmp), gb, p.dims[0], s)) return e;
      }
    }
    return 0;
  }

  int gated_backward(const Op& c) {
    const OpDesc& o = c.o;
    const int h = kG.head[c.i], P_slots = epi_partials(c.dm);
    const GateBlock blk = gate_block(c);
    SseBwdIn g{written[o.dst] ? at(p.grad[o.dst]) : nullptr, nullptr, c.lv == 0 ? g_pred[h] : fat(p.glvl[h][c.lv])};
    SseHead hd = sse_head(c.i, false);
    float* g_head = head_slice(c.i, grads).gw;
    if (p.d.n_classes > 1) {
      if (int e = level_to_side_grad(c, g.g_level)) return e;
      g.g_level = nullptr;
      g.g_side = fat(p.gside);
      hd.side_out = nullptr;
      g_head = nullptr;
    }
    mark("epi_bwd:", o.name);
    if (int e = launch_sse_bwd_sums(p.d.dtype, blk, g, hd, SseSums{dat(p.stats), fat(p.pgrad)}, c.dm, s)) return e;
    mark("stats");
    const WgReduceJob rider = take_pending();
    if (int e = launch_gate_bwd_finalize(dat(p.stats), P_slots, c.r.cout, c.dm.N, c.dm.vox(), fat(p.m1), fat(p.m2), fat(p.pgrad),
                                         c.dm.N * P_slots, gpar(c.i, P_SE), gpar(c.i, P_SE2), gpar(c.i, P_CONV2_W),
                                         gpar(c.i, P_CONV2_B), g_head, s, &rider)) return e;
    mark("in_bwd:", o.name);
    if (int e = launch_sse_bwd_apply(p.d.dtype, blk, g, hd, SseApply{fat(p.m1), fat(p.m2), at(p.grad[o.dst])}, c.dm, s)) return e;
    written[o.dst] = true;
    if (float* gb = gpar(c.i, P_CONV1_B)) { zero_ptrs.push_back(gb); zero_counts.push_back(c.r.cout); }
    return conv_backward(c);
  }

  int cat_backward(const Op& c) {
    const OpDesc& o = c.o;
    const OpRes& r = c.r;
    const int P_slots = epi_partials(c.dm);
    SEUNET_CHECK(written[o.dst], "net: internal: gradient of %s output missing", o.name);
    const CatBlock blk = cat_block(c);
    const bool two = blk.b.kind != Branch2::None, recomputed = blk.b.kind == Branch2::Recomputed;
    float* gxw = two ? grads[kG.prm[c.i].xw] : nullptr;
    const void* g_out = at(p.grad[o.dst]);
    PoolGrad pool{};
    if (r.fused >= 0) pool = PoolGrad{reinterpret_cast<const unsigned*>(at(p.op[r.fused].pool_idx)), at(p.grad[kOps[r.fused].dst])};
    mark("cat_bwd:", o.name);
    const CatSums sums{dat(p.stats), dat(p.stats2), recomputed && gxw ? dat(p.xwp) : nullptr};
    if (int e = launch_cat_bwd_sums(p.d.dtype, blk, g_out, pool, sums, c.dm, s)) return e;
    mark("stats");
    const CatXwFinalize xwf{dat(p.xwp), dat(r.xtot), blk.b.w2, p.d.in_channel, p.d.eps, recomputed ? gxw : nullptr};
    const WgReduceJob rider = take_pending();
    if (int e = launch_cat_bwd_finalize(dat(p.stats), two ? dat(p.stats2) : nullptr, P_slots, r.cout, c.dm.N, c.dm.vox(), fat(p.m1),
                                        fat(p.m2), fat(p.m1b), fat(p.m2b), xwf, s, &rider)) return e;
    mark("in_bwd:", o.name);
    CatApply ap{fat(p.m1), fat(p.m2), fat(p.m1b), fat(p.m2b), at(p.grad[o.dst]), two && !recomputed ? at(p.gx) : nullptr, nullptr, 0};
    if (recomputed && grad_x) { ap.gx_out = gxl(c.lv); ap.gx_acc = c.lv == 1 ? 1 : 0; }
    if (int e = launch_cat_bwd_apply(p.d.dtype, blk, g_out, pool, ap, c.dm, s)) return e;
    if (two && !recomputed) {
      if (grad_x) {
        mark("input_grad:", o.xname);
        if (int e = launch_xgrad_contract(p.d.dtype, at(p.gx), r.cout, par(kG.prm[c.i].xw), p.d.in_channel, gxl(c.lv), c.lv == 1 ? 1 : 0, c.dm, s)) return e;
      }
      if (gxw) {
        mark("wgrad:", o.xname);
        if (int e = walk_wgrad(r.x_wgrad, 1, 1, xbranch_src(o), p.d.in_channel, at(p.gx), r.cout, gxw, c.dm)) return e;
      }
    }
    return conv_backward(c);
  }

  int pool_backward(const Op& c) {
    const OpDesc& o = c.o;
    const int t = o.src[0];
    if (grad_x && o.dst == T_X2) {
      mark("input_grad:unpool1");
      if (int e = launch_xgrad_unpool(p.d.dtype, at(p.feat[T_X1]), p.d.in_channel, gxl(2), gxl(1), p.dims[1], s)) return e;
    }
    if (is_input(t)) return 0;
    SEUNET_CHECK(written[o.dst], "net: internal: gradient of %s output missing", o.name);
    mark("pool_bwd:", o.name);
    if (c.r.fused >= 0) {
      SEUNET_CHECK(written[t], "net: internal: gradient of %s input missing before its deferred pool gradient", o.name);
      return 0;
    }
    if (int e = launch_maxpool_bwd(p.d.dtype, at(p.feat[t]), at(p.grad[o.dst]), p.C[t], at(p.grad[t]), written[t] ? 1 : 0,
                                   p.dims_of(t), s)) return e;
    written[t] = true;
    return 0;
  }

  int up_backward(const Op& c) {
    const int t = c.o.src[0];
    SEUNET_CHECK(written[c.o.dst], "net: internal: gradient of %s output missing", c.o.name);
    mark("up_bwd:", c.o.name);
    if (int e = launch_upsample2_bwd(p.d.dtype, at(p.grad[c.o.dst]), p.C[t], at(p.grad[t]), written[t] ? 1 : 0, p.dims_of(t), s)) return e;
    written[t] = true;
    return 0;
  }

  int backward(const float* g_pred0, const float* g_pred1, const float* drop1, const float* drop2, float* const* grads_) {
    drops[0] = drop1; drops[1] = drop2;
    g_pred[0] = g_pred0; g_pred[1] = g_pred1;
    grads = grads_;
    if (int e = pack_all_weights(true)) return e;
    if (int e = heads_backward()) return e;
    for (int i = kNumOps - 1; i >= 0; --i) {
      if (decoder_done && i == kG.first_up) {
        if (int e = flush_pending()) return e;
        SEUNET_HIP(hipEventRecord(decoder_done, s));
      }
      const Op c = op(i);
      const OpKind k = c.o.kind;
      if (int e = k == OP_GATED ? gated_backward(c) : k == OP_CAT ? cat_backward(c) : k == OP_POOL ? pool_backward(c) : up_backward(c))
        return e;
    }
    if (!zero_ptrs.empty() || pending.blocks() > 0) {
      mark("stats");
      const WgReduceJob rider = take_pending();
      if (int e = launch_multi_zero(zero_ptrs.data(), zero_counts.data(), (int)zero_ptrs.size(), s, &rider)) return e;
    }
    if (grad_x) {
      mark("input_grad:ec1");
      if (int e = launch_input_grad(p.d.dtype, at(p.grad[T_E0]), p.C[T_E0], par(0, P_CONV1_W), at(p.feat[T_X0]), p.d.in_channel,
                                    gxl(0), gxl(1), grad_x, p.dims[0], s)) return e;
    }
    mark("outside");
    return 0;
  }
};

}
}

using namespace seunet;

extern "C" {

int seunet_net_param_count(const seunet_net_desc* desc) {
  return desc ? kNumParams : -1;
}

int seunet_net_param_info(const seunet_net_desc* desc, int index, char* name, int name_cap, int* shape5, int* ndim) {
  SEUNET_CHECK(desc && name && shape5 && ndim, "param_info: null argument");
  SEUNET_CHECK(index >= 0 && index < kNumParams, "param_info: index %d out of range", index);
  const seunet_net_desc& d = *desc;
  const ParamDesc& q = kG.param[index];
  snprintf(name, (size_t)name_cap, "%s.%s", q.block, kFieldName[q.f]);
  const int ci = q.cin ? q.cin * d.width_mult : d.in_channel, co = q.cout * d.width_mult;
  const int shapes[][5] = {{co, ci, q.k, q.k, q.k}, {co}, {2, co, 1, 1, 1}, {2}, {1, co, 1, 1, 1}, {1, co, 1, 1, 1},
                           {d.n_classes, q.cin, 1, 1, 1}, {d.n_classes}};
  for (int k = 0; k < 5; ++k) shape5[k] = shapes[q.f][k];
  *ndim = shapes[q.f][1] ? 5 : 1;
  return 0;
}

size_t seunet_net_workspace_bytes(const seunet_net_desc* desc) {
  Plan p;
  return desc && p.init(*desc) == 0 ? p.total : 0;
}

int seunet_debug_net_layout(const seunet_net_desc* desc, int index, char* name, int cap, size_t* offset, size_t* bytes) {
  SEUNET_CHECK(desc && name && offset && bytes, "debug_net_layout: null argument");
  Plan p;
  if (int e = p.init(*desc)) return e;
  if (index < 0 || index >= (int)p.log.size()) return 1;
  const Take& t = p.log[index];
  snprintf(name, (size_t)cap, "%s%s%s", t.what, t.of[0] ? ":" : "", t.of);
  *offset = t.off;
  *bytes = t.bytes;
  return 0;
}

int seunet_debug_net_wgrad_defer(int on) {
  const int was = g_wgrad_defer ? 1 : 0;
  g_wgrad_defer = on != 0;
  return was;
}

int seunet_net_forward(const seunet_net_desc* desc, const float* const* params, const float* x, const float* drop1,
                       const float* drop2, float* pred0, float* pred1, void* workspace, size_t workspace_bytes,
                       seunet_stream_t s) {
  SEUNET_CHECK(x && pred1, "net_forward: null tensor");
  Exec ex;
  if (int e = ex.setup(desc, params, workspace, workspace_bytes, (hipStream_t)s)) return e;
  return ex.forward(x, drop1, drop2, pred0, pred1);
}

struct NetGraph {
  hipGraph_t graph = nullptr;
  hipGraphExec_t exec = nullptr;
};

int seunet_net_forward_capture(const seunet_net_desc* desc, const float* const* params, const float* x, const float* drop1,
                               const float* drop2, float* pred0, float* pred1, void* workspace, size_t workspace_bytes,
                               seunet_stream_t s, void** graph_out) {
  SEUNET_CHECK(x && pred1 && graph_out, "net_forward_capture: null argument");
  SEUNET_CHECK(s != nullptr, "net_forward_capture: stream capture needs a stream other than the null stream");
  SEUNET_CHECK(!prof_on(), "net_forward_capture: switch the launch-group timer off before capturing");
  *graph_out = nullptr;
  Exec ex;
  if (int e = ex.setup(desc, params, workspace, workspace_bytes, (hipStream_t)s)) return e;
  SEUNET_CHECK(device_zero_page() != nullptr, "net_forward_capture: zero page allocation failed");
  SEUNET_HIP(hipStreamBeginCapture((hipStream_t)s, hipStreamCaptureModeThreadLocal));
  const int rc = ex.forward(x, drop1, drop2, pred0, pred1);
  NetGraph* g = new NetGraph;
  const hipError_t e_end = hipStreamEndCapture((hipStream_t)s, &g->graph);
  if (rc != 0 || e_end != hipSuccess) {
    if (g->graph) (void)hipGraphDestroy(g->graph);
    delete g;
    if (rc != 0) return rc;
    return fail("net_forward_capture: hipStreamEndCapture failed: %s", hipGetErrorString(e_end));
  }
  const hipError_t e_inst = hipGraphInstantiate(&g->exec, g->graph, nullptr, nullptr, 0);
  if (e_inst != hipSuccess) {
    (void)hipGraphDestroy(g->graph);
    delete g;
    return fail("net_forward_capture: hipGraphInstantiate failed: %s", hipGetErrorString(e_inst));
  }
  *graph_out = g;
  return 0;
}

int seunet_graph_launch(void* graph, seunet_stream_t s) {
  SEUNET_CHECK(graph != nullptr, "graph_launch: null graph");
  SEUNET_HIP(hipGraphLaunch(static_cast<NetGraph*>(graph)->exec, (hipStream_t)s));
  return 0;
}

int seunet_graph_destroy(void* graph) {
  if (!graph) return 0;
  NetGraph* g = static_cast<NetGraph*>(graph);
  if (g->exec) (void)hipGraphExecDestroy(g->exec);
  if (g->graph) (void)hipGraphDestroy(g->graph);
  delete g;
  return 0;
}

int seunet_net_read_tensor(const seunet_net_desc* desc, const float* const* params, const void* workspace, size_t workspace_bytes,
                           const char* name, int which, float* out, int* channels, seunet_stream_t s) {
  SEUNET_CHECK(desc && workspace && name && out, "net_read_tensor: null argument");
  Plan p;
  int i;
  bool xbranch;
  if (int e = plan_and_find(*desc, -1, name, &p, &i, &xbranch)) return e;
  SEUNET_CHECK(workspace_bytes >= p.total, "net_read_tensor: workspace too small");
  SEUNET_CHECK(i >= 0, "net_read_tensor: no block named %s", name);
  const unsigned char* ws = reinterpret_cast<const unsigned char*>(workspace);
  const OpDesc& o = kOps[i];
  const OpRes& r = p.op[i];
  const Dims& dm = p.dims_of(o.dst);
  const size_t raw = xbranch ? r.raw2 : r.raw, mean = xbranch ? r.mean2 : r.mean, rstd = xbranch ? r.rstd2 : r.rstd;
  SEUNET_CHECK(!xbranch || (which >= 0 && which <= 2), "net_read_tensor: which=%d is not stored for an x-branch", which);
  if (channels) *channels = which == 3 ? p.C[o.dst] : r.cout;
  if (xbranch && which == 0 && p.fuse_x) {
    SEUNET_CHECK(params != nullptr, "net_read_tensor: the recomputed x-branch %s needs the parameter list", name);
    const float* w = params[kG.prm[i].xw];
    SEUNET_CHECK(w, "net_read_tensor: no weight for %s", name);
    return launch_xbranch_values(p.d.dtype, ws + p.feat[o.xsrc], w, r.cout, p.d.in_channel, out, dm, (hipStream_t)s);
  }
// ... 85 lines not shown
```

se-unet-airseg_amd/csrc/wgrad.h:

```cpp
#pragma once
#include "seunet_common.h"

namespace seunet {

struct WgReduceJob;

bool wgrad_stream_supported(int dtype, int taps, int dil, int x_c, int dy_c);
size_t wgrad_stream_workspace_bytes(int x_c, int dy_c, int dil, Dims d);
int launch_wgrad_stream(int dtype, int dil, const void* x, int x_c, int cin_w, const void* dy, int dy_c, int cout_w, float* dw,
                        void* workspace, size_t ws_bytes, Dims d, hipStream_t s, WgReduceJob* defer = nullptr);

static constexpr int WG_TILED_SLABS = 512;
size_t wgrad_workspace_bytes(int taps, int cin, int cout);
int launch_wgrad(int dtype, int taps, int dil, const SrcList& x, int cin_logical, const void* dy,
                 int cout, float* dw_torch, void* workspace, size_t ws_bytes, Dims d, hipStream_t s, WgReduceJob* defer = nullptr);
bool wgrad_march_supported(int dtype, int taps, int dil, const SrcList& x, int cin_logical, int cout, Dims d, long long src_dist);
int launch_wgrad_march(int dtype, int taps, int dil, const SrcList& x, int cin_logical, const void* dy, int cout,
                       float* dw, void* workspace, size_t ws_bytes, Dims d, hipStream_t s, WgReduceJob* defer = nullptr);
size_t wgrad_march_workspace_bytes(int taps, int cin, int cout);
bool wgrad_1x1_supported(int dtype, const SrcList& x, int cin_logical, int cout);
int launch_wgrad_1x1(int dtype, const SrcList& x, int cin_logical, const void* dy, int cout, float* dw, void* workspace,
                     size_t ws_bytes, Dims d, hipStream_t s, WgReduceJob* defer = nullptr);
size_t wgrad_1x1_workspace_bytes(int cin, int cout);
int launch_wgrad_naive(int dtype, int taps, int dil, const SrcList& x, int cin_logical,
                       const void* dy, int cout, float* dw_torch, Dims d, hipStream_t s);
ConvKernel wgrad_kernel(int dtype, int taps, int dil, const SrcList& x, int cin_logical, int cout, Dims d, long long src_dist);
int run_wgrad(ConvKernel k, int dtype, int taps, int dil, const SrcList& x, int cin_logical, const void* dy, int cout, float* dw,
              void* workspace, size_t ws_bytes, Dims d, hipStream_t s, WgReduceJob* defer = nullptr);

static constexpr size_t WG_SLAB_PREFIX = 256;
struct WgSlabs {
  size_t prefix, nslab, per;
  size_t bytes() const { return prefix + nslab * per * sizeof(float); }
  float* base(void* workspace, size_t ws_bytes) const {
    return ws_bytes >= bytes() ? reinterpret_cast<float*>(reinterpret_cast<unsigned char*>(workspace) + prefix) : nullptr;
  }
};

#ifdef __HIPCC__
struct WgMap {
  int taps, cin_w, cout_w, co_tiles;
  __device__ long long operator()(int combo, int e) const {
    const int tap = e >> 10, ci = (combo / co_tiles) * 32 + ((e >> 5) & 31), co = (combo % co_tiles) * 32 + (e & 31);
    return ci < cin_w && co < cout_w ? (long long)(((size_t)co * cin_w + ci) * taps + tap) : -1;
  }
};
struct WmMap {
  int ncb, pw, xc, yc, nco, cin_w;
  __device__ long long operator()(int combo, int e) const {
    const int comp = e & 3, lane = (e >> 2) & 63, tap = (e >> 8) % 27, pair = e / (27 * 256);
    const int wave = pair / pw, kk = pair % pw;
    const int cib = wave % ncb, cob = (wave / ncb) * pw + kk;
    const int co = (combo % nco) * yc + cob * 16 + 4 * (lane >> 4) + comp;
    const int ci = (combo / nco) * xc + cib * 16 + (lane & 15);
    return (long long)(((size_t)co * cin_w + ci) * 27 + tap);
  }
};
struct WsMap {
  int cin, cout, cin_w, cout_w;
  __device__ long long operator()(int, int e) const {
    const int co = e % cout, ci = (e / cout) % cin, tap = e / (cout * cin);
    return ci < cin_w && co < cout_w ? (long long)(((size_t)co * cin_w + ci) * 27 + tap) : -1;
  }
};
struct W1Map {
  int cibw, ncob, cin;
  __device__ long long operator()(int, int e) const {
    const int comp = e & 3, lane = (e >> 2) & 63, pair = e >> 8;
    const int kk = pair % ncob, c = (pair / ncob) % cibw, wave = pair / (ncob * cibw);
    const int co = kk * 16 + 4 * (lane >> 4) + comp;
    const int ci = (wave * cibw + c) * 16 + (lane & 15);
    return ci < cin ? (long long)((size_t)co * cin + ci) : -1;
  }
};

struct WgReduceJob {
  enum Kind { None, Tiled, March, Stream, One } kind = None;
  const float* slab = nullptr;
  int nslab = 0, per = 0, combos = 0;
  float* dw = nullptr;
  union { WgMap g; WmMap m; WsMap s; W1Map o; } map = {};
  void set(const WgMap& v) { kind = Tiled; map.g = v; }
  void set(const WmMap& v) { kind = March; map.m = v; }
  void set(const WsMap& v) { kind = Stream; map.s = v; }
  void set(const W1Map& v) { kind = One; map.o = v; }
  __host__ __device__ int blocks_per_combo() const { return (per + 63) / 64; }
  int blocks() const { return kind == None ? 0 : combos * blocks_per_combo(); }
};

static constexpr int WG_RED_PAD = 65;
template <typename Map>
__device__ __forceinline__ void wgrad_reduce_elements(const float* __restrict__ slab, int nslab, int per, const Map& map,
                                                      float* __restrict__ dw, int bx, int combo, double (&red)[16][WG_RED_PAD]) {
  const int quad = threadIdx.x & 15, part = threadIdx.x >> 4;
  const int e0 = bx * 64 + quad * 4;
  double s0[4] = {0.0, 0.0, 0.0, 0.0}, s1[4] = {0.0, 0.0, 0.0, 0.0};
  if (e0 < per) {
    const float* p = slab + (size_t)combo * nslab * per + e0;
    int k = part;
    for (; k + 16 < nslab; k += 32) {
      const float4 a = *reinterpret_cast<const float4*>(p + (size_t)k * per);
      const float4 b = *reinterpret_cast<const float4*>(p + (size_t)(k + 16) * per);
      s0[0] += (double)a.x; s0[1] += (double)a.y; s0[2] += (double)a.z; s0[3] += (double)a.w;
      s1[0] += (double)b.x; s1[1] += (double)b.y; s1[2] += (double)b.z; s1[3] += (double)b.w;
    }
    if (k < nslab) {
      const float4 a = *reinterpret_cast<const float4*>(p + (size_t)k * per);
      s0[0] += (double)a.x; s0[1] += (double)a.y; s0[2] += (double)a.z; s0[3] += (double)a.w;
    }
  }
#pragma unroll
  for (int j = 0; j < 4; ++j) red[part][quad * 4 + j] = s0[j] + s1[j];
  __syncthreads();
  const int el = threadIdx.x, e = bx * 64 + el;
  if (el < 64 && e < per) {
    const long long i = map(combo, e);
    if (i >= 0) {
      double t = red[0][el];
#pragma unroll
      for (int q = 1; q < 16; ++q) t += red[q][el];
      dw[i] = (float)t;
    }
  }
}

__device__ __forceinline__ void wgrad_reduce_body(const WgReduceJob& job, int block) {
  __shared__ double red[16][WG_RED_PAD];
  const int bpc = job.blocks_per_combo();
  const int combo = block / bpc, bx = block % bpc;
  switch (job.kind) {
    case WgReduceJob::Tiled: wgrad_reduce_elements(job.slab, job.nslab, job.per, job.map.g, job.dw, bx, combo, red); break;
    case WgReduceJob::March: wgrad_reduce_elements(job.slab, job.nslab, job.per, job.map.m, job.dw, bx, combo, red); break;
    case WgReduceJob::Stream: wgrad_reduce_elements(job.slab, job.nslab, job.per, job.map.s, job.dw, bx, combo, red); break;
    case WgReduceJob::One: wgrad_reduce_elements(job.slab, job.nslab, job.per, job.map.o, job.dw, bx, combo, red); break;
    default: break;
  }
}

int launch_wgrad_reduce(const WgReduceJob& job, hipStream_t s);
template <typename Map>
static int finish_wgrad(const float* slab, int nslab, int per, int combos, const Map& map, float* dw, WgReduceJob* defer,
                        hipStream_t s) {
  SEUNET_CHECK(per % 4 == 0 && (reinterpret_cast<uintptr_t>(slab) & 15) == 0,
               "wgrad: the slab reduction reads 16 bytes at a time (slab of %d floats at %p)", per, (const void*)slab);
  WgReduceJob job;
  job.slab = slab; job.nslab = nslab; job.per = per; job.combos = combos; job.dw = dw;
  job.set(map);
  if (defer) { *defer = job; return 0; }
  return launch_wgrad_reduce(job, s);
}
#endif

}
```

se-unet-airseg_amd/ops.py:

```python
from __future__ import annotations

import ctypes as C
from typing import List, Optional, Sequence, Tuple

import torch

from . import _lib
from ._lib import Dims


def _tdtype(code: int):
    return {_lib.BF16: torch.bfloat16, _lib.F16: torch.float16}.get(code, torch.float32)


def _code(t: torch.Tensor) -> int:
    return {torch.bfloat16: _lib.BF16, torch.float16: _lib.F16}.get(t.dtype, _lib.F32)


def _dims_cl(t: torch.Tensor) -> Dims:
    n, d, h, w, _ = t.shape
    return Dims(n, d, h, w)


def _s():
# ... 256 lines not shown
    def call(m1, m2, m1b, m2b, o1, o2, s1, s2):
        _lib.check(lib.seunet_cat_epilogue_bwd(_code(raw), g_out.data_ptr(), raw.data_ptr(), mean.data_ptr(), rstd.data_ptr(),
                                               _lib.ptr(raw2), _lib.ptr(mean2), _lib.ptr(rstd2), c, slope, _lib.ptr(m1), _lib.ptr(m2),
                                               _lib.ptr(m1b), _lib.ptr(m2b), _lib.ptr(o1), _lib.ptr(o2), _lib.ptr(s1), _lib.ptr(s2),
                                               dims, _s()), "cat_epilogue_bwd")
    call(None, None, None, None, None, None, st, st2)
    m1, m2 = stats_finalize(st, slots, d * h * w, 0.0, 1)
    m1b, m2b = stats_finalize(st2, slots, d * h * w, 0.0, 1) if raw2 is not None else (None, None)
    call(m1, m2, m1b, m2b, dx, dx2, None, None)
    return dx, dx2


def xbranch_stats(x_in, w2, in_channel, eps=1e-5):
    lib = _lib.load()
    n, d, h, w, _ = x_in.shape
    dims = _dims_cl(x_in)
    c = w2.shape[0]
    w2f = w2.contiguous().float().reshape(c, in_channel)
    mslots = lib.seunet_xbranch_moment_slots(dims)
    mom = torch.zeros((n, mslots, 5), dtype=torch.float64, device=x_in.device)
    _lib.check(lib.seunet_xbranch_moments(_code(x_in), x_in.data_ptr(), mom.data_ptr(), dims, _s()), "xbranch_moments")
    mean2 = torch.empty((n, c), dtype=torch.float32, device=x_in.device)
    rstd2 = torch.empty_like(mean2)
    tot = torch.empty((n, 5), dtype=torch.float64, device=x_in.device)
    _lib.check(lib.seunet_xbranch_stats(mom.data_ptr(), mslots, w2f.data_ptr(), c, in_channel, n, d * h * w, eps, mean2.data_ptr(),
                                        rstd2.data_ptr(), tot.data_ptr(), _s()), "xbranch_stats")
    return mean2, rstd2, tot


def cat_epilogue_fwd_x(raw, mean, rstd, x_in, w2, in_channel, mean2, rstd2, slope=0.01):
    c = raw.shape[4]
    w2f = w2.contiguous().float().reshape(c, in_channel)
    out = torch.empty_like(raw)
    _lib.check(_lib.load().seunet_cat_epilogue_fwd_x(_code(raw), raw.data_ptr(), mean.data_ptr(), rstd.data_ptr(), x_in.data_ptr(),
                                                     w2f.data_ptr(), in_channel, mean2.data_ptr(), rstd2.data_ptr(), c, slope,
                                                     out.data_ptr(), _dims_cl(raw), _s()), "cat_epilogue_fwd_x")
    return out


def cat_epilogue_fwd_x_pool(raw, mean, rstd, x_in, w2, in_channel, mean2, rstd2, slope=0.01):
    n, d, h, w, c = raw.shape
    w2f = w2.contiguous().float().reshape(c, in_channel)
    out = torch.empty_like(raw)
    pooled = torch.empty((n, d // 2, h // 2, w // 2, c), dtype=raw.dtype, device=raw.device)
    words = torch.empty((n, (d // 2) * (h // 2) * (w // 2), c // 8), dtype=torch.int32, device=raw.device)
    _lib.check(_lib.load().seunet_cat_epilogue_fwd_x_pool(_code(raw), raw.data_ptr(), mean.data_ptr(), rstd.data_ptr(), x_in.data_ptr(),
                                                          w2f.data_ptr(), in_channel, mean2.data_ptr(), rstd2.data_ptr(), c, slope,
                                                          out.data_ptr(), pooled.data_ptr(), words.data_ptr(), _dims_cl(raw), _s()),
               "cat_epilogue_fwd_x_pool")
    return out, pooled, words


def cat_epilogue_bwd_x(g_out, raw, mean, rstd, x_in, w2, in_channel, mean2, rstd2, moments, slope=0.01, eps=1e-5,
                       pool_argmax=None, pool_g=None):
    lib = _lib.load()
    n, d, h, w, c = raw.shape
    dims = _dims_cl(raw)
    w2f = w2.contiguous().float().reshape(c, in_channel)
    slots = lib.seunet_epilogue_slots(dims)
    st = torch.zeros((n, slots, c, 2), dtype=torch.float64, device=raw.device)
    st2 = torch.zeros_like(st)
    part = torch.empty((n, slots, c, 2), dtype=torch.float64, device=raw.device)
    dx = torch.empty_like(raw)

    def bwd(m1, m2, m1b, m2b, o, s1, s2, xp):
        head = (_code(raw), g_out.data_ptr(), raw.data_ptr(), mean.data_ptr(), rstd.data_ptr(), x_in.data_ptr(), w2f.data_ptr(),
                in_channel, mean2.data_ptr(), rstd2.data_ptr(), c, slope, _lib.ptr(m1), _lib.ptr(m2), _lib.ptr(m1b), _lib.ptr(m2b),
                _lib.ptr(o), _lib.ptr(s1), _lib.ptr(s2), _lib.ptr(xp))
        if pool_argmax is None:
            _lib.check(lib.seunet_cat_epilogue_bwd_x(*head, dims, _s()), "cat_epilogue_bwd_x")
        else:
            _lib.check(lib.seunet_cat_epilogue_bwd_x_pool(*head, pool_argmax.data_ptr(), _lib.ptr(pool_g), dims, _s()),
                       "cat_epilogue_bwd_x_pool")
    bwd(None, None, None, None, None, st, st2, part)
    m1, m2 = stats_finalize(st, slots, d * h * w, 0.0, 1)
    m1b, m2b = stats_finalize(st2, slots, d * h * w, 0.0, 1)
    bwd(m1, m2, m1b, m2b, dx, None, None, None)
    dw = torch.zeros((c, in_channel, 1, 1, 1), dtype=torch.float32, device=raw.device)
    _lib.check(lib.seunet_cat_xgrad_finalize(part.data_ptr(), st2.data_ptr(), slots, moments.data_ptr(), w2f.data_ptr(), c,
                                             in_channel, n, eps, dw.data_ptr(), _s()), "cat_xgrad_finalize")
    return {"dx": dx, "dw2": dw, "m1": m1, "m2": m2, "m1b": m1b, "m2b": m2b}


def cat_epilogue_x(g_out, raw, mean, rstd, x_in, w2, in_channel, slope=0.01, eps=1e-5):
    mean2, rstd2, moments = xbranch_stats(x_in, w2, in_channel, eps)
    out = cat_epilogue_fwd_x(raw, mean, rstd, x_in, w2, in_channel, mean2, rstd2, slope)
    res = cat_epilogue_bwd_x(g_out, raw, mean, rstd, x_in, w2, in_channel, mean2, rstd2, moments, slope, eps)
    return out, res["dx"], res["dw2"]


def maxpool_fwd(t):
    n, d, h, w, c = t.shape
    out = torch.empty((n, d // 2, h // 2, w // 2, c), dtype=t.dtype, device=t.device)
    _lib.check(_lib.load().seunet_maxpool_fwd(_code(t), t.data_ptr(), c, out.data_ptr(), _dims_cl(t), _s()), "maxpool_fwd")
    return out


def maxpool_bwd(t, g_out, g_in=None):
    acc = 0 if g_in is None else 1
    g_in = torch.empty_like(t) if g_in is None else g_in
    _lib.check(_lib.load().seunet_maxpool_bwd(_code(t), t.data_ptr(), g_out.data_ptr(), t.shape[4], g_in.data_ptr(), acc,
                                              _dims_cl(t), _s()), "maxpool_bwd")
    return g_in


def upsample2_fwd(t):
    n, d, h, w, c = t.shape
    out = torch.empty((n, 2 * d, 2 * h, 2 * w, c), dtype=t.dtype, device=t.device)
    _lib.check(_lib.load().seunet_upsample2_fwd(_code(t), t.data_ptr(), c, out.data_ptr(), _dims_cl(t), _s()), "upsample2_fwd")
    return out


def upsample2_bwd(g_out, g_in=None):
    n, d2, h2, w2, c = g_out.shape
    acc = 0 if g_in is None else 1
    if g_in is None:
        g_in = torch.empty((n, d2 // 2, h2 // 2, w2 // 2, c), dtype=g_out.dtype, device=g_out.device)
    _lib.check(_lib.load().seunet_upsample2_bwd(_code(g_out), g_out.data_ptr(), c, g_in.data_ptr(), acc,
                                                Dims(n, d2 // 2, h2 // 2, w2 // 2), _s()), "upsample2_bwd")
    return g_in


def side_upsample(side: torch.Tensor, scale: int) -> torch.Tensor:
    n, d, h, w, c = side.shape
    out = torch.empty((n, c, d * scale, h * scale, w * scale), dtype=torch.float32, device=side.device)
    _lib.check(_lib.load().seunet_side_upsample(side.data_ptr(), c, scale, out.data_ptr(), c, 0, Dims(n, d, h, w), _s()),
               "side_upsample")
    return out


def head_fwd(level_maps: Sequence[torch.Tensor], bias: torch.Tensor) -> torch.Tensor:
    n, d, h, w = level_maps[0].shape
    pred = torch.empty((n, 1, d, h, w), dtype=torch.float32, device=bias.device)
    b = bias.contiguous().float()
    _lib.check(_lib.load().seunet_head_fwd(_lib.ptr_array(list(level_maps)), len(level_maps), b.data_ptr(), pred.data_ptr(),
                                           Dims(n, d, h, w), _s()), "head_fwd")
    return pred


def head_bwd(g_pred: torch.Tensor, nlevels: int):
    lib = _lib.load()
    n, _, d, h, w = g_pred.shape
    dims = Dims(n, d, h, w)
    g_pred = g_pred.contiguous().float()
    levels: List[Optional[torch.Tensor]] = [None]
    for l in range(1, nlevels):
        levels.append(torch.empty((n, d >> l, h >> l, w >> l), dtype=torch.float32, device=g_pred.device))
    tmp = torch.empty(lib.seunet_head_bwd_tmp_floats(dims), dtype=torch.float32, device=g_pred.device)
    gb = torch.empty(1, dtype=torch.float32, device=g_pred.device)
    _lib.check(lib.seunet_head_bwd(g_pred.data_ptr(), _lib.ptr_array(levels), nlevels, tmp.data_ptr(), gb.data_ptr(), dims, _s()),
               "head_bwd")
    return levels, gb


def _block_dtype():
    from .SE_UNet import _default_dtype
    return _lib.dtype_code(_default_dtype())


def _conv_stats(srcs, weight, bias, dilation, impl, cin=None):
    (raw,), part, slots = conv3d(srcs, weight, bias, dilation, impl, cin=cin, want_stats=True)
    n, d, h, w, _ = raw.shape
    mean, rstd = stats_finalize(part, slots, d * h * w)
    return raw, mean, rstd


# ... 78 lines not shown
```

Baseline: 582.4 million.

## Fuse cat block epilogue backward with 1x1 conv dgrad and wgrad GEMM

Adds a fused kernel for the concat block's backward pass. It applies the norm and leaky-ReLU backward (with optional maxpool gradient), then computes the 1x1 conv input gradients and weight-gradient partials with MFMA, using a multi-stage LDS DMA pipeline. The fused path is used only for the listed block dc22, when the shapes are supported and the workspace fits. It is meant to avoid materialising the pre-conv gradient and the separate passes over memory, at the cost of more LDS and register pressure and a new deferred reduce kind.

Result: no change. 585.2 million, median of 5 (+0.5%).

```diff
diff --git a/include/seunet_hip.h b/include/seunet_hip.h
--- a/include/seunet_hip.h
+++ b/include/seunet_hip.h
@@ -106,6 +106,14 @@
                                    const unsigned int* pool_argmax, const void* pool_g, seunet_dims dims, seunet_stream_t s);
 int seunet_cat_xgrad_finalize(const double* xw_partial, const double* stat_partial2, int slots, const double* moments,
                               const float* w2, int c, int in_channel, int n, float eps, float* dw, seunet_stream_t s);
+
+int seunet_cat_gemm_bwd_supported(int dtype, int nsrc, const int* src_c, int c, int pooled, seunet_dims dims);
+size_t seunet_cat_gemm_bwd_workspace_bytes(int cin, int c);
+int seunet_cat_gemm_bwd(int dtype, const void* g_out, const void* raw, const float* mean, const float* rstd, int c, float slope,
+                        const float* m1, const float* m2, const unsigned int* pool_argmax, const void* pool_g, int nsrc,
+                        const void* const* src, const int* src_c, const float* w, void* const* gx, const int* gx_accumulate,
+                        float* dw, void* workspace, size_t workspace_bytes, int max_groups, void* draw_out, seunet_dims dims,
+                        seunet_stream_t s);
 
 int seunet_maxpool_fwd(int dtype, const void* in, int c, void* out, seunet_dims in_dims, seunet_stream_t s);
 int seunet_maxpool_bwd(int dtype, const void* in, const void* g_out, int c, void* g_in, int accumulate,
diff --git a/se-unet-airseg_amd/_lib.py b/se-unet-airseg_amd/_lib.py
--- a/se-unet-airseg_amd/_lib.py
+++ b/se-unet-airseg_amd/_lib.py
@@ -107,6 +107,9 @@
     "seunet_cat_epilogue_bwd_x": (_i, [_i, _vp, _vp, _vp, _vp, _vp, _vp, _i, _vp, _vp, _i, _f, _vp, _vp, _vp, _vp, _vp, _vp, _vp, _vp, Dims, _vp]),
     "seunet_cat_epilogue_fwd_x_pool": (_i, [_i, _vp, _vp, _vp, _vp, _vp, _i, _vp, _vp, _i, _f, _vp, _vp, _vp, Dims, _vp]),
     "seunet_cat_epilogue_bwd_x_pool": (_i, [_i, _vp, _vp, _vp, _vp, _vp, _vp, _i, _vp, _vp, _i, _f, _vp, _vp, _vp, _vp, _vp, _vp, _vp, _vp, _vp, _vp, Dims, _vp]),
+    "seunet_cat_gemm_bwd_supported": (_i, [_i, _i, _ip, _i, _i, Dims]),
+    "seunet_cat_gemm_bwd_workspace_bytes": (_sz, [_i, _i]),
+    "seunet_cat_gemm_bwd": (_i, [_i, _vp, _vp, _vp, _vp, _i, _f, _vp, _vp, _vp, _vp, _i, _pp, _ip, _vp, _pp, _ip, _vp, _vp, _sz, _i, _vp, Dims, _vp]),
     "seunet_cat_xgrad_finalize": (_i, [_vp, _vp, _i, _vp, _vp, _i, _i, _i, _f, _vp, _vp]),
     "seunet_cc_workspace_bytes": (_sz, [_i, _i, _i]),
     "seunet_largest_component": (_i, [_vp, _i, _i, _i, _i, _vp, _vp, _vp, _sz, _vp]),
diff --git a/se-unet-airseg_amd/csrc/abi.cpp b/se-unet-airseg_amd/csrc/abi.cpp
--- a/se-unet-airseg_amd/csrc/abi.cpp
+++ b/se-unet-airseg_amd/csrc/abi.cpp
@@ -241,6 +241,28 @@
   return cat_epilogue_bwd(dtype, b, g_out, PoolGrad{}, m1, m2, m1b, m2b, dx, dx2, stat_partial, stat_partial2, nullptr, dims, s);
 }
 
+int seunet_cat_gemm_bwd_supported(int dtype, int nsrc, const int* src_c, int c, int pooled, seunet_dims dims) {
+  if (nsrc < 1 || nsrc > 3 || !src_c) return 0;
+  SrcList sl{};
+  sl.n = nsrc;
+  for (int i = 0; i < nsrc; ++i) sl.C[i] = src_c[i];
+  return cat_gemm_supported(dtype, sl, c, pooled != 0, D(dims)) ? 1 : 0;
+}
+size_t seunet_cat_gemm_bwd_workspace_bytes(int cin, int c) { return cat_gemm_workspace_bytes(cin, c); }
+int seunet_cat_gemm_bwd(int dtype, const void* g_out, const void* raw, const float* mean, const float* rstd, int c, float slope,
+                        const float* m1, const float* m2, const unsigned int* pool_argmax, const void* pool_g, int nsrc,
+                        const void* const* src, const int* src_c, const float* w, void* const* gx, const int* gx_accumulate, float* dw,
+                        void* workspace, size_t workspace_bytes, int max_groups, void* draw_out, seunet_dims dims, seunet_stream_t s) {
+  SrcList sl; DstList dl;
+  if (int e = make_src(nsrc, src, src_c, sl)) return e;
+  SEUNET_CHECK(gx != nullptr, "cat_gemm_bwd: null destination list");
+  if (int e = make_dst(nsrc, gx, src_c, gx_accumulate, dl)) return e;
+  SEUNET_CHECK((pool_argmax == nullptr) == (pool_g == nullptr), "cat_gemm_bwd: pool_argmax and pool_g go together");
+  const CatBlock b{{raw, mean, rstd}, {Branch2::None, nullptr, nullptr, nullptr, nullptr, 0}, c, slope};
+  return launch_cat_gemm_bwd(dtype, b, g_out, PoolGrad{pool_argmax, pool_g}, m1, m2, sl, w, dl, dw, workspace, workspace_bytes, max_groups,
+                             draw_out, D(dims), S(s));
+}
+
 int seunet_maxpool_fwd(int dtype, const void* in, int c, void* out, seunet_dims d, seunet_stream_t s) {
   SEUNET_CHECK(in && out, "maxpool_fwd: null tensor");
   return launch_maxpool_fwd(dtype, in, c, out, D(d), S(s));
diff --git a/se-unet-airseg_amd/csrc/cat.hip b/se-unet-airseg_amd/csrc/cat.hip
--- a/se-unet-airseg_amd/csrc/cat.hip
+++ b/se-unet-airseg_amd/csrc/cat.hip
@@ -110,27 +110,6 @@
   }
 }
 
-struct PoolRef {
-  const unsigned* argmax;
-  const void* g_pool;
-  unsigned W, H, Wo, Ho;
-  unsigned mW, mH;
-  long long Vo;
-};
-__device__ __forceinline__ unsigned div_small(unsigned n, unsigned d, unsigned m, unsigned& rem) {
-  unsigned q = __umulhi(n, m);
-  unsigned r = n - q * d;
-  if (r >= d) { ++q; r -= d; }
-  rem = r;
-  return q;
-}
-__device__ __forceinline__ void pool_locate(const PoolRef& pr, unsigned v, unsigned& kpos, unsigned& cv) {
-  unsigned x, y;
-  const unsigned t = div_small(v, pr.W, pr.mW, x);
-  const unsigned z = div_small(t, pr.H, pr.mH, y);
-  kpos = ((z & 1u) << 2) | ((y & 1u) << 1) | (x & 1u);
-  cv = ((z >> 1) * pr.Ho + (y >> 1)) * pr.Wo + (x >> 1);
-}
 
 template <typename T, int LPV, bool TWO, bool APPLY, bool XW, bool XR, bool XG>
 __global__ void __launch_bounds__(EPI_THREADS)
@@ -432,7 +411,7 @@
   return 0;
 }
 
-static int cat_bwd_pool(const char* who, bool xr, const PoolGrad& pool, Dims d, PoolRef& pr) {
+int cat_bwd_pool(const char* who, bool xr, const PoolGrad& pool, Dims d, PoolRef& pr) {
   pr = PoolRef{};
   if (pool.argmax == nullptr) return 0;
   SEUNET_CHECK(xr && pool.g_pool != nullptr && d.D % 2 == 0 && d.H % 2 == 0 && d.W % 2 == 0 && d.vox() < (1ll << 31),
diff --git a/se-unet-airseg_amd/csrc/cat_gemm.hip b/se-unet-airseg_amd/csrc/cat_gemm.hip
--- /dev/null
+++ b/se-unet-airseg_amd/csrc/cat_gemm.hip
@@ -0,0 +1,424 @@
+#include "epilogue.h"
+#include "lds_dma.h"
+#include "mfma.h"
+#include "wgrad.h"
+
+namespace seunet {
+
+struct CgArgs {
+  const void* src[3]; void* dst[3]; int srcC[3]; int acc[3]; int nsrc;
+  const void* raw; const void* g;
+  const float *mean, *rstd, *m1, *m2; float slope;
+  PoolRef pool;
+  const float* w; int cin;
+  float* slab; const void* zero; void* draw_out;
+  long long V; int nchunk;
+  int lw;
+};
+
+static constexpr int CG_NW = 4, CG_NST = 3, CG_PF = CG_NST - 1, CG_MAXI = 12;
+
+__device__ __forceinline__ int cg_swz(int np, int v) { return np >= 4 ? tr16_swz(np, v) : 0; }
+
+template <typename T, int CIBW, int NCOB, int DGB, bool POOL>
+__global__ void __launch_bounds__(256)
+cat_gemm_kernel(CgArgs a) {
+  constexpr int COUT = NCOB * 16, NP = COUT / 8, CH = 4096 / COUT, KS = CH / 32;
+  extern __shared__ __attribute__((aligned(16))) unsigned char smem[];
+  const unsigned lds_base = (unsigned)(size_t)(__attribute__((address_space(3))) unsigned char*)smem;
+  const int tid = threadIdx.x, lane = tid & 63;
+  const int wave = __builtin_amdgcn_readfirstlane(tid >> 6);
+  const int grp = lane >> 4, li = lane & 15, q = li >> 2, p = li & 3;
+  const int C0 = a.srcC[0], C1 = a.nsrc > 1 ? a.srcC[1] : 0, C2 = a.nsrc > 2 ? a.srcC[2] : 0;
+  const int cin = C0 + C1 + C2;
+  const int roff1 = C0 * 2 * CH, roff2 = roff1 + C1 * 2 * CH;
+  const int raw_off = cin * 2 * CH, g_off = raw_off + COUT * 2 * CH, gp_off = g_off + COUT * 2 * CH, am_off = gp_off + COUT * 2 * CH;
+  const int stage = POOL ? am_off + CH * NP * 4 : gp_off;
+  const int out_base = CG_NST * stage;
+  const int dump = out_base + cin * 2 * CH;
+  const int zoff = dump + 1024;
+  if (tid < 16) reinterpret_cast<unsigned*>(smem + zoff)[tid] = 0u;
+  __syncthreads();
+
+  int bsrc[CIBW], bcl[CIBW], bn[CIBW];
+#pragma unroll
+  for (int c = 0; c < CIBW; ++c) {
+    int rem = wave * CIBW + c;
+    bsrc[c] = 0; bcl[c] = 0; bn[c] = 0;
+    bool found = false;
+    for (int s = 0; s < a.nsrc; ++s) {
+      const int Cs = a.srcC[s], nb = (Cs + 15) / 16;
+      if (!found && rem < nb) { bsrc[c] = s; bcl[c] = rem * 16; bn[c] = Cs - rem * 16 < 16 ? Cs - rem * 16 : 16; found = true; }
+      rem -= nb;
+    }
+  }
+  auto roff_of = [&](int s) __attribute__((always_inline)) { return s == 0 ? 0 : (s == 1 ? roff1 : roff2); };
+  auto c_of = [&](int s) __attribute__((always_inline)) { return s == 0 ? C0 : (s == 1 ? C1 : C2); };
+
+  unsigned xoff[CIBW][KS][2], yoff[NCOB][KS][2];
+  bool xzero[CIBW];
+#pragma unroll
+  for (int c = 0; c < CIBW; ++c) {
+    const int Cs = c_of(bsrc[c]), nps = Cs / 8;
+    const int piece = bcl[c] / 8 + (p >> 1);
+    xzero[c] = piece * 8 >= Cs;
+#pragma unroll
+    for (int ks = 0; ks < KS; ++ks)
+#pragma unroll
+      for (int r = 0; r < 2; ++r) {
+        const int v = 32 * ks + 8 * grp + 4 * r + q;
+        xoff[c][ks][r] = (unsigned)(roff_of(bsrc[c]) + v * Cs * 2 + ((piece ^ cg_swz(nps, v)) * 16) + (p & 1) * 8);
+      }
+  }
+#pragma unroll
+  for (int k = 0; k < NCOB; ++k)
+#pragma unroll
+    for (int ks = 0; ks < KS; ++ks)
+#pragma unroll
+      for (int r = 0; r < 2; ++r) {
+        const int v = 32 * ks + 8 * grp + 4 * r + q;
+        yoff[k][ks][r] = (unsigned)(g_off + v * COUT * 2 + (((k * 2 + (p >> 1)) ^ tr16_swz(NP, v)) * 16) + (p & 1) * 8);
+      }
+
+  constexpr int VT32 = CH / 32, WPV = CG_NW / VT32, NBW = DGB;
+  const int dvt = wave / WPV;
+  const int row32 = lane & 31, hh = lane >> 5;
+  int dsrc[NBW], dcl[NBW], dn[NBW];
+  bf16x8 wf[NBW][COUT / 16];
+#pragma unroll
+  for (int nb = 0; nb < NBW; ++nb) {
+    int rem = (wave % WPV) * NBW + nb, gch0 = 0;
+    dsrc[nb] = 0; dcl[nb] = 0; dn[nb] = 0;
+    bool found = false;
+    int gbase = 0;
+    for (int s = 0; s < a.nsrc; ++s) {
+      const int Cs = a.srcC[s], nb32 = (Cs + 31) / 32;
+      if (!found && rem < nb32) { dsrc[nb] = s; dcl[nb] = rem * 32; dn[nb] = Cs - rem * 32 < 32 ? Cs - rem * 32 : 32; gch0 = gbase + rem * 32; found = true; }
+      rem -= nb32;
+      gbase += Cs;
+    }
+    const bool ok = row32 < dn[nb];
+#pragma unroll
+    for (int kc = 0; kc < COUT / 16; ++kc) {
+      float wv[8];
+#pragma unroll
+      for (int j = 0; j < 8; ++j) wv[j] = ok ? a.w[(size_t)(kc * 16 + 8 * hh + j) * cin + gch0 + row32] : 0.f;
+      u32x4 u;
+      u.x = pack2<T>(wv[0], wv[1]); u.y = pack2<T>(wv[2], wv[3]); u.z = pack2<T>(wv[4], wv[5]); u.w = pack2<T>(wv[6], wv[7]);
+      wf[nb][kc] = __builtin_bit_cast(bf16x8, u);
+    }
+  }
+
+  const int ni = stage / 1024;
+  const unsigned char* zero_page = reinterpret_cast<const unsigned char*>(a.zero) + lane * 16;
+  int kind[CG_MAXI];
+  unsigned step[CG_MAXI];
+  unsigned long long src[CG_MAXI];
+  static_for<CG_MAXI>([&](auto it_c) __attribute__((always_inline)) {
+    constexpr int it = decltype(it_c)::value;
+    const int id = wave + CG_NW * it, byte = id * 1024;
+    kind[it] = (it >= a.lw || id >= ni) ? 3 : (byte < gp_off ? 0 : (byte < am_off ? 1 : 2));
+    step[it] = 0; src[it] = 0;
+    if (kind[it] == 0) {
+      int C, rbase; const unsigned char* tb;
+      if (byte >= g_off) { C = COUT; rbase = g_off; tb = reinterpret_cast<const unsigned char*>(a.g); }
+      else if (byte >= raw_off) { C = COUT; rbase = raw_off; tb = reinterpret_cast<const unsigned char*>(a.raw); }
+      else if (a.nsrc > 2 && byte >= roff2) { C = C2; rbase = roff2; tb = reinterpret_cast<const unsigned char*>(a.src[2]); }
+      else if (a.nsrc > 1 && byte >= roff1) { C = C1; rbase = roff1; tb = reinterpret_cast<const unsigned char*>(a.src[1]); }
+      else { C = C0; rbase = 0; tb = reinterpret_cast<const unsigned char*>(a.src[0]); }
+      const int rel = byte - rbase + lane * 16;
+      const int sh = 31 - __clz(C * 2);
+      const int v = rel >> sh, slot = (rel & (C * 2 - 1)) >> 4;
+      src[it] = (unsigned long long)(size_t)(tb + (long long)blockIdx.x * CH * (C * 2) + (v << sh) + ((slot ^ cg_swz(C / 8, v)) * 16));
+      step[it] = (unsigned)(CH * C * 2) * gridDim.x;
+    } else if (kind[it] == 1) {
+      const int slot = (byte - gp_off) / 16 + lane;
+      src[it] = (unsigned long long)(unsigned)(slot / NP) | ((unsigned long long)(unsigned)((slot % NP) * 16) << 32);
+    } else if (kind[it] == 2) {
+      const int w4 = ((byte - am_off) / 16 + lane) * 4;
+      src[it] = (unsigned long long)(unsigned)(w4 / NP) | ((unsigned long long)(unsigned)((w4 % NP) * 4) << 32);
+    }
+  });
+  struct ChunkPos { long long n; long long vloc; };
+  const long long adv = (long long)gridDim.x * CH;
+  auto advance = [&](ChunkPos& c) __attribute__((always_inline)) {
+    c.vloc += adv;
+    while (c.vloc >= a.V) { c.vloc -= a.V; ++c.n; }
+  };
+  auto issue = [&](bool cok, const ChunkPos& c, int st) __attribute__((always_inline)) {
+    static_for<CG_MAXI>([&](auto it_c) __attribute__((always_inline)) {
+      constexpr int it = decltype(it_c)::value;
+      if (it < a.lw) {
+        const int id = wave + CG_NW * it;
+        const bool real = cok && kind[it] != 3;
+        const unsigned char* gp = zero_page;
+        if (kind[it] == 0) {
+          if (cok) gp = reinterpret_cast<const unsigned char*>((size_t)src[it]);
+          src[it] += step[it];
+        } else if (POOL && real) {
+          unsigned kpos, cv;
+          pool_locate(a.pool, (unsigned)c.vloc + (unsigned)src[it], kpos, cv);
+          const long long win = c.n * a.pool.Vo + cv;
+          gp = kind[it] == 1 ? reinterpret_cast<const unsigned char*>(a.pool.g_pool) + win * (COUT * 2) + (unsigned)(src[it] >> 32)
+                             : reinterpret_cast<const unsigned char*>(a.pool.argmax) + win * (NP * 4) + (unsigned)(src[it] >> 32);
+        }
+        dma16(gp, (unsigned)__builtin_amdgcn_readfirstlane((int)(real ? lds_base + (unsigned)(st * stage + id * 1024) : lds_base + (unsigned)dump)));
+      }
+    });
+  };
+
+  f32x4 acc[CIBW][NCOB];
+#pragma unroll
+  for (int c = 0; c < CIBW; ++c)
+#pragma unroll
+    for (int k = 0; k < NCOB; ++k) acc[c][k] = f32x4{0.f, 0.f, 0.f, 0.f};
+
+  const int cg = tid % NP, vb = tid / NP;
+  float mu[8], rs[8], a1[8], a2[8];
+  long long cur_n = -1;
+
+  int chunk = blockIdx.x, st = 0, stp = 0;
+  ChunkPos cur, nxt;
+  cur.n = ((long long)blockIdx.x * CH) / a.V;
+  cur.vloc = (long long)blockIdx.x * CH - cur.n * a.V;
+  nxt = cur;
+  for (int k = 0; k < CG_PF; ++k) {
+    issue(chunk + k * (int)gridDim.x < a.nchunk, nxt, stp);
+    advance(nxt);
+    stp = stp + 1 == CG_NST ? 0 : stp + 1;
+  }
+  auto store_image = [&](long long v0) __attribute__((always_inline)) {
+    for (int s = 0; s < a.nsrc; ++s) {
+      if (a.dst[s] == nullptr) continue;
+      const int Cs = c_of(s), np = CH * Cs / 8;
+      unsigned char* gdst = reinterpret_cast<unsigned char*>(a.dst[s]) + v0 * (Cs * 2);
+      const unsigned char* img = smem + out_base + roff_of(s);
+      const bool add = a.acc[s] != 0;
+      for (int i = tid; i < np; i += 256) {
+        Pack8<T> nw;
+        nw.u = *reinterpret_cast<const uint4*>(img + i * 16);
+        if (add) {
+          Pack8<T> old;
+          load8p(reinterpret_cast<const T*>(gdst + i * 16), old);
+          float x[8], y[8];
+          unpack8(nw, x);
+          unpack8(old, y);
+#pragma unroll
+          for (int j = 0; j < 8; ++j) x[j] += y[j];
+          store8(reinterpret_cast<T*>(gdst + i * 16), x);
+        } else {
+          *reinterpret_cast<uint4*>(gdst + i * 16) = nw.u;
+        }
+      }
+    }
+  };
+  long long prev_v0 = -1;
+  for (; chunk < a.nchunk; chunk += gridDim.x) {
+    if (a.lw == 8) wait_loads<(CG_PF - 1) * 8>(); else wait_loads<(CG_PF - 1) * 12>();
+    __builtin_amdgcn_s_barrier();
+    issue(chunk + CG_PF * (int)gridDim.x < a.nchunk, nxt, stp);
+    advance(nxt);
+    stp = stp + 1 == CG_NST ? 0 : stp + 1;
+    if (prev_v0 >= 0) store_image(prev_v0);
+    unsigned char* sp = smem + st * stage;
+    const unsigned sb = lds_base + (unsigned)(st * stage);
+    const long long v0 = (long long)chunk * CH;
+    const long long n = cur.n;
+    const unsigned vloc0 = (unsigned)cur.vloc;
+    advance(cur);
+
+    if (n != cur_n) {
+      cur_n = n;
+#pragma unroll
+      for (int j = 0; j < 8; ++j) {
+        const long long o = n * COUT + cg * 8 + j;
+        mu[j] = a.mean[o]; rs[j] = a.rstd[o]; a1[j] = a.m1[o]; a2[j] = a.m2[o];
+      }
+#pragma unroll
+      for (int j = 0; j < 8; ++j) asm volatile("" : "+v"(mu[j]), "+v"(rs[j]), "+v"(a1[j]), "+v"(a2[j]));
+    }
+#pragma unroll
+    for (int k = 0; k < 2; ++k) {
+      const int v = vb + k * (256 / NP);
+      const int po = v * COUT * 2 + ((cg ^ tr16_swz(NP, v)) * 16);
+      Pack8<T> pg, px;
+      pg.u = *reinterpret_cast<const uint4*>(sp + g_off + po);
+      px.u = *reinterpret_cast<const uint4*>(sp + raw_off + po);
+      float gy[8], x[8], d[8];
+      unpack8(pg, gy);
+      unpack8(px, x);
+      if (POOL) {
+        Pack8<T> pp;
+        pp.u = *reinterpret_cast<const uint4*>(sp + gp_off + (v * NP + cg) * 16);
+        const unsigned am = *reinterpret_cast<const unsigned*>(sp + am_off + (v * NP + cg) * 4);
+        unsigned kpos, cv;
+        pool_locate(a.pool, vloc0 + (unsigned)v, kpos, cv);
+        float gp[8];
+        unpack8(pp, gp);
+#pragma unroll
+        for (int j = 0; j < 8; ++j) gy[j] += ((am >> (3 * j)) & 7u) == kpos ? gp[j] : 0.f;
+      }
+#pragma unroll
+      for (int j = 0; j < 8; ++j) {
+        const float xh = (x[j] - mu[j]) * rs[j];
+        d[j] = gy[j] * lrelu_slope(xh, a.slope);
+        d[j] = rs[j] * (d[j] - a1[j] - xh * a2[j]);
+      }
+      uint4 u;
+      u.x = pack2<T>(d[0], d[1]); u.y = pack2<T>(d[2], d[3]); u.z = pack2<T>(d[4], d[5]); u.w = pack2<T>(d[6], d[7]);
+      *reinterpret_cast<uint4*>(sp + g_off + po) = u;
+      if (a.draw_out != nullptr)
+        *reinterpret_cast<uint4*>(reinterpret_cast<unsigned char*>(a.draw_out) + ((v0 + v) * COUT + cg * 8) * 2) = u;
+    }
+    asm volatile("s_waitcnt lgkmcnt(0)" ::: "memory");
+    __builtin_amdgcn_s_barrier();
+
+#pragma unroll
+    for (int ks = 0; ks < KS; ++ks) {
+      bf16x8 yf[NCOB];
+#pragma unroll
+      for (int k = 0; k < NCOB; ++k) yf[k] = frag_tr16(sb + yoff[k][ks][0], sb + yoff[k][ks][1]);
+#pragma unroll
+      for (int c = 0; c < CIBW; ++c) {
+        if (bn[c] > 0) {
+          const unsigned z = lds_base + (unsigned)zoff;
+          const bf16x8 xf = frag_tr16(xzero[c] ? z : sb + xoff[c][ks][0], xzero[c] ? z : sb + xoff[c][ks][1]);
+#pragma unroll
+          for (int k = 0; k < NCOB; ++k) acc[c][k] = mfma_16x16x32<T>(yf[k], xf, acc[c][k]);
+        }
+      }
+    }
+    {
+      const int v = dvt * 32 + row32;
+      bf16x8 df[COUT / 16];
+#pragma unroll
+      for (int kc = 0; kc < COUT / 16; ++kc)
+        df[kc] = __builtin_bit_cast(bf16x8, *reinterpret_cast<const u32x4*>(sp + g_off + v * COUT * 2 + (((kc * 2 + hh) ^ tr16_swz(NP, v)) * 16)));
+#pragma unroll
+      for (int nb = 0; nb < NBW; ++nb) {
+        if (dn[nb] > 0) {
+          f32x16 dg;
+#pragma unroll
+          for (int i = 0; i < 16; ++i) dg[i] = 0.f;
+#pragma unroll
+          for (int kc = 0; kc < COUT / 16; ++kc) dg = mfma_32x32x16<T>(wf[nb][kc], df[kc], dg);
+          const int s = dsrc[nb], Cs = c_of(s);
+#pragma unroll
+          for (int rg = 0; rg < 4; ++rg) {
+            const int cl = 8 * rg + 4 * hh;
+            u32x2 pk;
+            pk.x = pack2<T>(dg[4 * rg], dg[4 * rg + 1]); pk.y = pack2<T>(dg[4 * rg + 2], dg[4 * rg + 3]);
+            const int o = cl < dn[nb] ? out_base + roff_of(s) + v * Cs * 2 + (dcl[nb] + cl) * 2 : dump + lane * 8;
+            *reinterpret_cast<u32x2*>(smem + o) = pk;
+          }
+        }
+      }
+    }
+    asm volatile("s_waitcnt lgkmcnt(0)" ::: "memory");
+    prev_v0 = v0;
+    st = st + 1 == CG_NST ? 0 : st + 1;
+  }
+  wait_loads<0>();
+  __builtin_amdgcn_s_barrier();
+  store_image(prev_v0);
+
+  float* out = a.slab + ((size_t)blockIdx.x * CG_NW + wave) * (CIBW * NCOB * 256) + lane * 4;
+#pragma unroll
+  for (int c = 0; c < CIBW; ++c)
+#pragma unroll
+    for (int k = 0; k < NCOB; ++k) *reinterpret_cast<f32x4*>(out + (c * NCOB + k) * 256) = acc[c][k];
+}
+
+struct CgCfg { int cibw, ncob, ch, lw, lds, cin; WcMap map; };
+static bool cat_gemm_cfg(int dtype, const SrcList& x, int cout, bool pooled, Dims d, CgCfg& c) {
+  if (dtype_size(dtype) != 2 || x.n < 1 || x.n > 3 || (cout != 32 && cout != 64)) return false;
+  c = CgCfg{};
+  int nblk = 0, ch0 = 0, nb32 = 0;
+  for (int i = 0; i < x.n; ++i) {
+    const int C = x.C[i];
+    if (C != 8 && C != 16 && C != 32 && C != 64) return false;
+    nb32 += (C + 31) / 32;
+    for (int b = 0; b * 16 < C; ++b, ++nblk) {
+      if (nblk >= 16) return false;
+      c.map.blk_c0[nblk] = (unsigned char)(ch0 + b * 16);
+      c.map.blk_n[nblk] = (unsigned char)(C - b * 16 < 16 ? C - b * 16 : 16);
+    }
+    ch0 += C;
+  }
+  c.cin = ch0;
+  c.cibw = (nblk + CG_NW - 1) / CG_NW;
+  c.ncob = cout / 16;
+  if (!((c.cibw == 1 && c.ncob == 2) || (c.cibw == 2 && c.ncob == 2) || (c.cibw == 2 && c.ncob == 4))) return false;
+  c.map.cibw = c.cibw; c.map.ncob = c.ncob; c.map.cin = c.cin;
+  c.ch = 4096 / cout;
+  if (nb32 > (cout == 32 ? 3 : 4)) return false;
+  const long long V = d.vox();
+  if (d.N < 1 || V < c.ch || V % c.ch != 0 || (long long)d.N * V / c.ch > 0x7fffffffll / 4) return false;
+  if (pooled && (d.D % 2 || d.H % 2 || d.W % 2 || V >= (1ll << 31))) return false;
+  const int stage = (c.cin + 2 * cout) * 2 * c.ch + (pooled ? cout * 2 * c.ch + c.ch * (cout / 8) * 4 : 0);
+  const int items = (stage / 1024 + CG_NW - 1) / CG_NW;
+  if (stage % 1024 != 0 || items > CG_MAXI) return false;
+  c.lw = items <= 8 ? 8 : 12;
+  c.lds = CG_NST * stage + c.cin * 2 * c.ch + 1024 + 64;
+  return c.lds <= 160 * 1024;
+}
+bool cat_gemm_supported(int dtype, const SrcList& x, int cout, bool pooled, Dims d) {
+  CgCfg c;
+  return cat_gemm_cfg(dtype, x, cout, pooled, d, c);
+}
+
+static constexpr int CG_MAX_WG = 256;
+static WgSlabs cg_slabs(int groups, int cibw, int ncob) { return {WG_SLAB_PREFIX, (size_t)groups, (size_t)CG_NW * cibw * ncob * 256}; }
+size_t cat_gemm_workspace_bytes(int, int cout) { return cg_slabs(CG_MAX_WG, 2, cdiv(cout, 16)).bytes(); }
+
+template <typename T, int CIBW, int NCOB, int DGB, bool POOL>
+static int cat_gemm_launch(const CgArgs& a, int grid, int lds, hipStream_t s) {
+  static unsigned long long configured = 0;
+  if (int e = configure_kernel_lds(configured, reinterpret_cast<const void*>(&cat_gemm_kernel<T, CIBW, NCOB, DGB, POOL>), lds)) return e;
+  cat_gemm_kernel<T, CIBW, NCOB, DGB, POOL><<<grid, 256, lds, s>>>(a);
+  SEUNET_LAUNCH_CHECK();
+  return 0;
+}
+
+int launch_cat_gemm_bwd(int dtype, const CatBlock& b, const void* g_out, const PoolGrad& pool, const float* m1, const float* m2,
+                        const SrcList& x, const float* w, const DstList& gx, float* dw, void* workspace, size_t ws_bytes,
+                        int max_groups, void* draw_out, Dims d, hipStream_t s, WgReduceJob* defer) {
+  CgCfg c;
+  const bool pooled = pool.argmax != nullptr;
+  SEUNET_CHECK(cat_gemm_cfg(dtype, x, b.C, pooled, d, c),
+               "cat_gemm_bwd: 16-bit tensors, 1..3 sources of 8 / 16 / 32 / 64 channels (at most 8 blocks of 16), 32 or 64 output "
+               "channels, a voxel count per sample that is a multiple of %d, even extents with a pooled gradient", b.C ? 4096 / b.C : 0);
+  SEUNET_CHECK(b.b.kind != Branch2::Stored, "cat_gemm_bwd: a stored second branch needs pass B's second output");
+  SEUNET_CHECK(g_out && b.a.raw && b.a.mean && b.a.rstd && m1 && m2 && w && dw && workspace, "cat_gemm_bwd: missing argument");
+  SEUNET_CHECK(gx.n == x.n, "cat_gemm_bwd: one destination per source");
+  CgArgs a{};
+  for (int i = 0; i < x.n; ++i) {
+    SEUNET_CHECK(x.ptr[i] != nullptr && gx.C[i] == x.C[i], "cat_gemm_bwd: source %d missing, or its destination has other channels", i);
+    a.src[i] = x.ptr[i]; a.srcC[i] = x.C[i]; a.dst[i] = gx.ptr[i]; a.acc[i] = gx.ptr[i] ? gx.acc[i] : 0;
+  }
+  a.nsrc = x.n;
+  if (int e = cat_bwd_pool("cat_gemm_bwd", true, pool, d, a.pool)) return e;
+  a.raw = b.a.raw; a.g = g_out; a.mean = b.a.mean; a.rstd = b.a.rstd; a.m1 = m1; a.m2 = m2; a.slope = b.slope;
+  a.w = w; a.cin = c.cin;
+  a.zero = device_zero_page();
+  SEUNET_CHECK(a.zero != nullptr, "cat_gemm_bwd: cannot allocate the device zero page");
+  a.draw_out = draw_out;
+  a.V = d.vox();
+  a.nchunk = (int)((long long)d.N * a.V / c.ch);
+  a.lw = c.lw;
+  int grid = a.nchunk < CG_MAX_WG ? a.nchunk : CG_MAX_WG;
+  if (max_groups > 0 && max_groups < grid) grid = max_groups;
+  const WgSlabs slabs = cg_slabs(grid, c.cibw, c.ncob);
+  a.slab = slabs.base(workspace, ws_bytes);
+  SEUNET_CHECK(a.slab != nullptr, "cat_gemm_bwd: workspace too small");
+  int e = -1;
+  SEUNET_DTYPE_SWITCH(dtype, if constexpr (sizeof(T) == 2) {
+    if (c.cibw == 1) e = pooled ? cat_gemm_launch<T, 1, 2, 3, true>(a, grid, c.lds, s) : cat_gemm_launch<T, 1, 2, 3, false>(a, grid, c.lds, s);
+    else if (c.ncob == 2) e = pooled ? cat_gemm_launch<T, 2, 2, 3, true>(a, grid, c.lds, s) : cat_gemm_launch<T, 2, 2, 3, false>(a, grid, c.lds, s);
+    else e = pooled ? cat_gemm_launch<T, 2, 4, 2, true>(a, grid, c.lds, s) : cat_gemm_launch<T, 2, 4, 2, false>(a, grid, c.lds, s);
+  });
+  if (e) return e;
+  return finish_wgrad(a.slab, grid, (int)slabs.per, 1, c.map, dw, defer, s);
+}
+
+}
diff --git a/se-unet-airseg_amd/csrc/epilogue.h b/se-unet-airseg_amd/csrc/epilogue.h
--- a/se-unet-airseg_amd/csrc/epilogue.h
+++ b/se-unet-airseg_amd/csrc/epilogue.h
@@ -54,6 +54,14 @@
 struct CatBlock { NormIn a; Branch2 b; int C; float slope; };
 struct PoolOut { void* pooled; unsigned* argmax; };
 struct PoolGrad { const unsigned* argmax; const void* g_pool; };
+struct PoolRef {
+  const unsigned* argmax;
+  const void* g_pool;
+  unsigned W, H, Wo, Ho;
+  unsigned mW, mH;
+  long long Vo;
+};
+int cat_bwd_pool(const char* who, bool xr, const PoolGrad& pool, Dims d, PoolRef& pr);
 struct CatSums {
   double* stat_partial;
   double* stat_partial2;
@@ -81,6 +89,11 @@
 int launch_cat_bwd_finalize(const double* stat_partial, const double* stat_partial2, int slots, int C, int N, long long count,
                             float* m1, float* m2, float* m1b, float* m2b, const CatXwFinalize& xw, hipStream_t s,
                             const WgReduceJob* rider = nullptr);
+bool cat_gemm_supported(int dtype, const SrcList& x, int cout, bool pooled, Dims d);
+size_t cat_gemm_workspace_bytes(int cin, int cout);
+int launch_cat_gemm_bwd(int dtype, const CatBlock& b, const void* g_out, const PoolGrad& pool, const float* m1, const float* m2,
+                        const SrcList& x, const float* w, const DstList& gx, float* dw, void* workspace, size_t ws_bytes,
+                        int max_groups, void* draw_out, Dims d, hipStream_t s, WgReduceJob* defer = nullptr);
 int launch_xbranch_values(int dtype, const void* x_in, const float* w2, int C, int in_channel, float* out_ncdhw, Dims d, hipStream_t s);
 
 #ifdef __HIPCC__
@@ -105,6 +118,21 @@
 __device__ __forceinline__ float lrelu(float xh, float slope) { return xh > 0.f ? xh : xh * slope; }
 __device__ __forceinline__ float norm_lrelu(float x, float mu, float rs, float slope) { return lrelu((x - mu) * rs, slope); }
 __device__ __forceinline__ float lrelu_slope(float xh, float slope) { return xh > 0.f ? 1.f : slope; }
+
+__device__ __forceinline__ unsigned div_small(unsigned n, unsigned d, unsigned m, unsigned& rem) {
+  unsigned q = __umulhi(n, m);
+  unsigned r = n - q * d;
+  if (r >= d) { ++q; r -= d; }
+  rem = r;
+  return q;
+}
+__device__ __forceinline__ void pool_locate(const PoolRef& pr, unsigned v, unsigned& kpos, unsigned& cv) {
+  unsigned x, y;
+  const unsigned t = div_small(v, pr.W, pr.mW, x);
+  const unsigned z = div_small(t, pr.H, pr.mH, y);
+  kpos = ((z & 1u) << 2) | ((y & 1u) << 1) | (x & 1u);
+  cv = ((z >> 1) * pr.Ho + (y >> 1)) * pr.Wo + (x >> 1);
+}
 
 template <typename E, int K> __device__ __forceinline__ E wave4_sum(const E (&red)[4][16][K], int g, int k) {
   return ((red[0][g][k] + red[1][g][k]) + red[2][g][k]) + red[3][g][k];
diff --git a/se-unet-airseg_amd/csrc/net.cpp b/se-unet-airseg_amd/csrc/net.cpp
--- a/se-unet-airseg_amd/csrc/net.cpp
+++ b/se-unet-airseg_amd/csrc/net.cpp
@@ -26,6 +26,8 @@
 namespace {
 
 bool g_wgrad_defer = true;
+bool g_cat_gemm = true;
+constexpr const char* kCatGemmBlocks[] = {"dc22"};
 
 enum TId {
   T_NONE,
@@ -189,6 +191,20 @@
     return kG.nsrc[i] == 2 ? (long long)feat[kOps[i].src[1]] - (long long)feat[kOps[i].src[0]] : 0;
   }
 
+  bool cat_gemm_route(int i, bool input_grad) const {
+    const OpDesc& o = kOps[i];
+    const OpRes& r = op[i];
+    if (!g_cat_gemm || o.kind != OP_CAT || input_grad || d.conv_impl == SEUNET_CONV_NAIVE || !r.need_dgrad) return false;
+    if (o.xname && !fuse_x) return false;
+    bool listed = false;
+    for (const char* b : kCatGemmBlocks) listed = listed || strcmp(b, o.name) == 0;
+    if (!listed) return false;
+    SrcList x{};
+    x.n = kG.nsrc[i];
+    for (int k = 0; k < x.n; ++k) x.C[k] = C[o.src[k]];
+    return cat_gemm_supported(d.dtype, x, r.cout, r.fused >= 0, dims_of(o.dst)) && cat_gemm_workspace_bytes(r.cin, r.cout) <= wgrad_ws_bytes;
+  }
+
   void route(int i) {
     const OpDesc& o = kOps[i];
     OpRes& r = op[i];
@@ -681,6 +697,23 @@
     const WgReduceJob rider = take_pending();
     if (int e = launch_cat_bwd_finalize(dat(p.stats), two ? dat(p.stats2) : nullptr, P_slots, r.cout, c.dm.N, c.dm.vox(), fat(p.m1),
                                         fat(p.m2), fat(p.m1b), fat(p.m2b), xwf, s, &rider)) return e;
+    float* gw = gpar(c.i, P_CONV1_W);
+    if (gw && p.cat_gemm_route(c.i, grad_x != nullptr)) {
+      const SrcList x = srcs(c.i);
+      DstList gd{};
+      gd.n = x.n;
+      for (int k = 0; k < x.n; ++k) {
+        const int t = o.src[k];
+        gd.C[k] = p.C[t];
+        gd.ptr[k] = is_input(t) ? nullptr : at(p.grad[t]);
+        gd.acc[k] = (!is_input(t) && written[t]) ? 1 : 0;
+        if (!is_input(t)) written[t] = true;
+      }
+      if (int e = flush_pending()) return e;
+      mark("cat_gemm_bwd:", o.name);
+      return launch_cat_gemm_bwd(p.d.dtype, blk, g_out, pool, fat(p.m1), fat(p.m2), x, par(c.i, P_CONV1_W), gd, gw, at(p.wgrad_ws),
+                                 p.wgrad_ws_bytes, 0, nullptr, c.dm, s, defer());
+    }
     mark("in_bwd:", o.name);
     CatApply ap{fat(p.m1), fat(p.m2), fat(p.m1b), fat(p.m2b), at(p.grad[o.dst]), two && !recomputed ? at(p.gx) : nullptr, nullptr, 0};
     if (recomputed && grad_x) { ap.gx_out = gxl(c.lv); ap.gx_acc = c.lv == 1 ? 1 : 0; }
@@ -804,6 +837,21 @@
   const int was = g_wgrad_defer ? 1 : 0;
   g_wgrad_defer = on != 0;
   return was;
+}
+
+int seunet_debug_net_cat_gemm(int on) {
+  const int was = g_cat_gemm ? 1 : 0;
+  g_cat_gemm = on != 0;
+  return was;
+}
+int seunet_debug_net_cat_gemm_route(const seunet_net_desc* desc, int input_grad, const char* name) {
+  if (!desc || !name) { (void)fail("debug_net_cat_gemm_route: null argument"); return -1; }
+  Plan p;
+  if (p.init(*desc) != 0) return -1;
+  for (int i = 0; i < kNumOps; ++i)
+    if (strcmp(kOps[i].name, name) == 0) return p.cat_gemm_route(i, input_grad != 0) ? 1 : 0;
+  (void)fail("debug_net_cat_gemm_route: no block named %s", name);
+  return -1;
 }
 
 int seunet_net_forward(const seunet_net_desc* desc, const float* const* params, const float* x, const float* drop1,
diff --git a/se-unet-airseg_amd/csrc/wgrad.h b/se-unet-airseg_amd/csrc/wgrad.h
--- a/se-unet-airseg_amd/csrc/wgrad.h
+++ b/se-unet-airseg_amd/csrc/wgrad.h
@@ -73,17 +73,29 @@
     return ci < cin ? (long long)((size_t)co * cin + ci) : -1;
   }
 };
+struct WcMap {
+  int cibw, ncob, cin;
+  unsigned char blk_c0[16], blk_n[16];
+  __device__ long long operator()(int, int e) const {
+    const int comp = e & 3, lane = (e >> 2) & 63, pair = e >> 8;
+    const int kk = pair % ncob, c = (pair / ncob) % cibw, wave = pair / (ncob * cibw);
+    const int co = kk * 16 + 4 * (lane >> 4) + comp;
+    const int b = wave * cibw + c, cl = lane & 15;
+    return cl < (int)blk_n[b] ? (long long)((size_t)co * cin + blk_c0[b] + cl) : -1;
+  }
+};
 
 struct WgReduceJob {
-  enum Kind { None, Tiled, March, Stream, One } kind = None;
+  enum Kind { None, Tiled, March, Stream, One, Cat } kind = None;
   const float* slab = nullptr;
   int nslab = 0, per = 0, combos = 0;
   float* dw = nullptr;
-  union { WgMap g; WmMap m; WsMap s; W1Map o; } map = {};
+  union { WgMap g; WmMap m; WsMap s; W1Map o; WcMap c; } map = {};
   void set(const WgMap& v) { kind = Tiled; map.g = v; }
   void set(const WmMap& v) { kind = March; map.m = v; }
   void set(const WsMap& v) { kind = Stream; map.s = v; }
   void set(const W1Map& v) { kind = One; map.o = v; }
+  void set(const WcMap& v) { kind = Cat; map.c = v; }
   __host__ __device__ int blocks_per_combo() const { return (per + 63) / 64; }
   int blocks() const { return kind == None ? 0 : combos * blocks_per_combo(); }
 };
@@ -133,6 +145,7 @@
     case WgReduceJob::March: wgrad_reduce_elements(job.slab, job.nslab, job.per, job.map.m, job.dw, bx, combo, red); break;
     case WgReduceJob::Stream: wgrad_reduce_elements(job.slab, job.nslab, job.per, job.map.s, job.dw, bx, combo, red); break;
     case WgReduceJob::One: wgrad_reduce_elements(job.slab, job.nslab, job.per, job.map.o, job.dw, bx, combo, red); break;
+    case WgReduceJob::Cat: wgrad_reduce_elements(job.slab, job.nslab, job.per, job.map.c, job.dw, bx, combo, red); break;
     default: break;
   }
 }
diff --git a/se-unet-airseg_amd/ops.py b/se-unet-airseg_amd/ops.py
--- a/se-unet-airseg_amd/ops.py
+++ b/se-unet-airseg_amd/ops.py
@@ -362,6 +362,34 @@
     return {"dx": dx, "dw2": dw, "m1": m1, "m2": m2, "m1b": m1b, "m2b": m2b}
 
 
+def cat_gemm_bwd_supported(code, src_channels, c, pooled, dims) -> bool:
+    return bool(_lib.load().seunet_cat_gemm_bwd_supported(code, len(src_channels), _lib.int_array(list(src_channels)), c, int(pooled),
+                                                          Dims(*dims)))
+
+
+def cat_gemm_bwd(g_out, raw, mean, rstd, m1, m2, srcs, weight, slope=0.01, pool_argmax=None, pool_g=None, gx=None, accumulate=None,
+                 max_groups=0, want_draw=False, workspace=None):
+    lib = _lib.load()
+    n, d, h, w, c = raw.shape
+    dims = _dims_cl(raw)
+    chans = [t.shape[4] for t in srcs]
+    cin = sum(chans)
+    wf = weight.contiguous().float().reshape(c, cin)
+    if gx is None:
+        gx = [torch.empty_like(t) for t in srcs]
+    accumulate = list(accumulate or [0] * len(srcs))
+    dw = torch.empty((c, cin, 1, 1, 1), dtype=torch.float32, device=raw.device)
+    if workspace is None:
+        workspace = torch.empty(lib.seunet_cat_gemm_bwd_workspace_bytes(cin, c), dtype=torch.uint8, device=raw.device)
+    draw = torch.empty_like(raw) if want_draw else None
+    _lib.check(lib.seunet_cat_gemm_bwd(_code(raw), g_out.data_ptr(), raw.data_ptr(), mean.data_ptr(), rstd.data_ptr(), c, slope,
+                                       m1.data_ptr(), m2.data_ptr(), _lib.ptr(pool_argmax), _lib.ptr(pool_g), len(srcs),
+                                       _lib.ptr_array(list(srcs)), _lib.int_array(chans), wf.data_ptr(), _lib.ptr_array(list(gx)),
+                                       _lib.int_array(accumulate), dw.data_ptr(), workspace.data_ptr(), workspace.numel(), max_groups,
+                                       _lib.ptr(draw), dims, _s()), "cat_gemm_bwd")
+    return {"gx": list(gx), "dw": dw, "draw": draw}
+
+
 def cat_epilogue_x(g_out, raw, mean, rstd, x_in, w2, in_channel, slope=0.01, eps=1e-5):
     mean2, rstd2, moments = xbranch_stats(x_in, w2, in_channel, eps)
     out = cat_epilogue_fwd_x(raw, mean, rstd, x_in, w2, in_channel, mean2, rstd2, slope)
```
